# leejaeyong7/nerfacc

Hardware: AMD Instinct MI355X
Metric: rays/sec (fwd+bwd) through 128^3 occ-grid, 1M-ray batch (higher is better)
Workload: dtype f32; 1 GPU; cfg2: 1048576 image rays/GPU, 128^3 shell10 occ grid (G=1), step 2*sqrt(3)/1024, sampling+rendering fwd+bwd; rays_per_gpu=1048576, resolution=128, grid=shell10, samples_after_compaction=32244949, parallelism=ray-sharded x1, field=synthetic analytic field, native callbacks (see bench.py NativeField/TorchField)

## Files before the change

include/nerfacc_hip.h:

```cpp
#ifndef NERFACC_HIP_H
#define NERFACC_HIP_H

#include <stdint.h>

#ifdef __cplusplus
extern "C" {
#endif

#define NFA_OK 0
#define NFA_EINVAL (-1)
#define NFA_EHIP (-2)

#define NFA_MAX_GRID_LEVELS 8

typedef void *nfa_stream_t;

#define NFA_ELEM_F32 0
#define NFA_ELEM_F16 1
#define NFA_ELEM_BF16 2

const char *nfa_last_error(void);
#define NFA_VERSION 403
int nfa_version(void);
int nfa_set_tuning(const char *name, const char *value);
int nfa_device_arch(char *buf, int buflen);


int64_t nfa_cumsum_scratch_bytes(int64_t n);
int nfa_exclusive_cumsum_i64(const int64_t *cnts, int64_t n, int64_t *starts, int64_t *total,
                             void *scratch, nfa_stream_t stream);
int nfa_exclusive_cumsum_pairs_i64(const int64_t *cnts, int64_t n, int64_t *packed_info , int64_t *total,
                                   void *scratch, nfa_stream_t stream);
int nfa_exclusive_cumsum_pairs_stats_i64(const int64_t *cnts, int64_t n, int64_t *packed_info ,
                                         int64_t *total_and_stats , void *scratch, nfa_stream_t stream);

int nfa_pack_info(const int64_t *ray_indices, int64_t n, int64_t n_rays, int64_t *packed_info ,
                  int32_t *flags , void *scratch, nfa_stream_t stream);

int nfa_unpack_rows(const void *packed, const int64_t *packed_info , const uint8_t *mask, int64_t n_rays,
                    int64_t n_per_ray, int64_t n_packed, int64_t row_bytes, const void *pad_host, int32_t pad_bytes,
                    void *padded, nfa_stream_t stream);
int nfa_pack_rows(const void *padded, const int64_t *packed_info , const uint8_t *mask, int64_t n_rays,
                  int64_t n_per_ray, int64_t n_packed, int64_t row_bytes, void *packed, nfa_stream_t stream);
int nfa_mask_row_counts(const uint8_t *mask, int64_t n_rows, int64_t n_cols, int64_t *counts, nfa_stream_t stream);

int nfa_pack_bits(const uint8_t *binaries, int64_t n_cells, uint32_t *bits , nfa_stream_t stream);


int nfa_ray_aabb_intersect(const float *rays_o, const float *rays_d, int64_t n_rays,
                           const float *aabbs, int32_t n_aabbs, float near_plane, float far_plane,
                           float miss_value, float *t_mins, float *t_maxs, uint8_t *hits,
                           nfa_stream_t stream);

#define NFA_MAX_EVENT_LEVELS 8
int nfa_ray_events(const float *rays_o, const float *rays_d, int64_t n_rays, const float *aabbs, int32_t n_aabbs,
                   float *t_sorted, int64_t *t_indices, uint8_t *hits, nfa_stream_t stream);

typedef struct nfa_traverse_args {
    int64_t n_rays;
    const float *rays_o;
    const float *rays_d;
    const uint8_t *rays_mask;
    int32_t n_grids;
    int32_t res[3];
    const uint8_t *binaries;
    const float *aabbs;
    const uint8_t *hits;
    const float *t_sorted;
    const int64_t *t_indices;
    const float *near_planes;
    const float *far_planes;
    float step_size;
    float cone_angle;
    int32_t traverse_steps_limit;
    int32_t mode;
    float *iv_vals; int64_t *iv_ray_indices; uint8_t *iv_is_left; uint8_t *iv_is_right;
    int64_t *iv_starts; int64_t *iv_cnts;
    float *sm_vals; int64_t *sm_ray_indices; uint8_t *sm_is_valid;
    float *sm_t_starts; float *sm_t_ends;
    int64_t *sm_starts; int64_t *sm_cnts;
    float *terminate_planes;
    const int32_t *ray_filter;
    int32_t ray_filter_min;
    const uint64_t *bricks;
    const uint32_t *coarse;
    const int32_t *steps_limit_dev;
    const int64_t *n_listed_dev;
    const int32_t *run_if_nonzero;
} nfa_traverse_args;
int nfa_traverse_grids(const nfa_traverse_args *args, nfa_stream_t stream);

int64_t nfa_bricks_words(int32_t n_grids, const int32_t *res);
int nfa_pack_bricks(const uint8_t *binaries, int32_t n_grids, const int32_t *res, uint64_t *bricks,
                    uint32_t *coarse, nfa_stream_t stream);
int64_t nfa_walk_bits_words(int32_t n_grids, const int32_t *res);
int nfa_pack_walk_bits(const uint8_t *binaries, int32_t n_grids, const int32_t *res, uint32_t *bits, nfa_stream_t stream);
int nfa_traverse_runs(const nfa_traverse_args *args, const uint32_t *bits, int32_t *run_cnts, uint64_t *runs,
                      int32_t max_runs, int32_t *overflow_count, float near_hint, const int32_t *ray_order,
                      int64_t n_order, nfa_stream_t stream);
int nfa_bin_rays(const float *rays_o, const float *rays_d, int64_t n_rays, const float *box, int32_t *order,
                 void *scratch, nfa_stream_t stream);
int nfa_alive_rays(const float *opacity, const int64_t *packed_info , int64_t n_samples, float opacity_max,
                   int64_t n_rays, uint8_t *mask, int32_t *alive, int64_t *count, nfa_stream_t stream);
int nfa_testmode_begin(int64_t *alive_count, int32_t *state, int64_t n_rays, int32_t min_samples, int32_t max_samples,
                       int64_t *sm_cnts, int32_t *run_cnts, int64_t *zero_words, int32_t n_zero, nfa_stream_t stream);
int nfa_testmode_alive(const float *opacity, const int64_t *packed_info, int32_t *state, float opacity_max, int64_t n_rays,
                       uint8_t *mask, int32_t *alive, int64_t *count, int32_t count_samples, nfa_stream_t stream);
int nfa_bin_rays_levels(const float *rays_o, const float *rays_d, int64_t n_rays, const float *aabbs, int32_t n_grids,
                        const int32_t *res, float near_plane, int32_t *order, void *scratch,
                        uint64_t *coherence , nfa_stream_t stream);
int nfa_expand_runs(int64_t n_rays, float step_size, const int32_t *run_cnts, const uint64_t *runs,
                    int32_t max_runs, const int64_t *packed_info , float *t_starts,
                    float *t_ends, float *t_mids, int64_t *ray_indices, int64_t capacity, nfa_stream_t stream);
int nfa_fill_ray_indices(int64_t n_rays, const int64_t *packed_info , int64_t *ray_indices,
                         nfa_stream_t stream);
int nfa_traverse_cone_runs(const nfa_traverse_args *args, int32_t *run_cnts, uint64_t *runs, int32_t max_runs,
                           int32_t *overflow_count, const int32_t *ray_order ,
                           int64_t n_order, nfa_stream_t stream);
int nfa_traverse_cone_walk(const nfa_traverse_args *args, const uint32_t *bits, int32_t *run_cnts, uint64_t *runs,
                           int32_t max_runs, int32_t *overflow_count, uint32_t *arena, int32_t arena_capacity,
                           const int32_t *ray_order, int64_t n_order, nfa_stream_t stream);
int nfa_expand_cone_arena(const uint32_t *arena, int32_t n_entries, float step_size, float cone_angle,
                          const int64_t *packed_info , float *t_starts, float *t_ends, int64_t *ray_indices,
                          nfa_stream_t stream);
int nfa_expand_cone_runs(int64_t n_rays, float step_size, float cone_angle, const int32_t *run_cnts,
                         const uint64_t *runs, int32_t max_runs, const int64_t *packed_info, float *t_starts,
                         float *t_ends, int64_t *ray_indices, nfa_stream_t stream);
int nfa_expand_intervals(int64_t n_rays, float step_size, const int32_t *run_cnts, const uint64_t *runs,
                         int32_t max_runs, const int64_t *iv_packed_info , float *vals,
                         int64_t *ray_indices, uint8_t *is_left, uint8_t *is_right, nfa_stream_t stream);


int nfa_grid_cell_points(const int64_t *indices, const float *jitter , int64_t n, const int32_t *res,
                         const float *aabb , float *x , nfa_stream_t stream);
int nfa_grid_ema_update(float *occs, int64_t cell_base, const int64_t *indices, int64_t n, const float *occ,
                        float ema_decay, float *scratch , nfa_stream_t stream);
int64_t nfa_grid_rebinarize_scratch_bytes(void);
int nfa_grid_rebinarize(const float *occs, int32_t n_grids, const int32_t *res, float occ_thre, uint8_t *binaries,
                        uint32_t *walk_bits, void *scratch, nfa_stream_t stream);


void nfa_seg_plan(int64_t n_elems, int64_t n_rays, int64_t *tile_elems, int64_t *n_tiles);
int64_t nfa_seg_table_rows(int64_t n_tiles);
int nfa_seg_build_tiles(const int64_t *packed_info , int64_t n_rays, int64_t n_elems,
                        int64_t tile_elems, int64_t n_tiles, int64_t *tiles ,
                        int32_t *flags, nfa_stream_t stream);

int nfa_packed_scan(int kind, int reverse, const int64_t *packed_info, const int64_t *tiles, int64_t n_tiles,
                    int64_t n_rays, int64_t n_elems, const float *inputs, float *outputs,
                    nfa_stream_t stream);
int nfa_packed_scan_generic(int kind, int reverse, int normalize, const int64_t *packed_info,
                            int64_t n_rays, int64_t n_elems, const float *inputs, float *outputs,
                            nfa_stream_t stream);
int nfa_packed_prod_backward(int kind, const int64_t *packed_info, const int64_t *tiles, int64_t n_tiles,
                             int64_t n_rays, int64_t n_elems, const float *inputs,
                             const float *outputs, const float *grad_outputs, float *grad_inputs,
                             nfa_stream_t stream);

int nfa_render_from_density_fwd(const float *t_starts, const float *t_ends, const float *sigmas,
                                const float *prefix_trans , const int64_t *packed_info,
                                const int64_t *tiles, int64_t n_tiles, int64_t n_rays, int64_t n_elems,
                                float *weights, float *trans, float *alphas, nfa_stream_t stream);
int nfa_render_from_alpha_fwd(const float *alphas, const float *prefix_trans, const int64_t *packed_info,
                              const int64_t *tiles, int64_t n_tiles, int64_t n_rays, int64_t n_elems,
                              float *weights, float *trans, nfa_stream_t stream);
int nfa_render_from_density_bwd(const float *t_starts, const float *t_ends, const float *trans,
                                const float *alphas, const float *g_weights, const float *g_trans,
                                const float *g_alphas, const int64_t *packed_info, const int64_t *tiles, int64_t n_tiles,
                                int64_t n_rays, int64_t n_elems, float *grad_sigmas, float *grad_x,
                                nfa_stream_t stream);
int nfa_density_cdf_rows_fwd(const float *t_starts, const float *t_ends, const float *sigmas, const int64_t *packed_info,
                             const int64_t *tiles, int64_t n_tiles, int64_t n_rays, int64_t n_elems, int32_t row_len,
                             float *trans, float *alphas, float *cdfs , nfa_stream_t stream);
int nfa_density_cdf_rows_bwd(const float *t_starts, const float *t_ends, const float *trans, const float *alphas,
                             const float *g_cdfs , const int64_t *packed_info, const int64_t *tiles,
                             int64_t n_tiles, int64_t n_rays, int64_t n_elems, int32_t row_len, float *grad_sigmas,
                             nfa_stream_t stream);
int nfa_render_from_alpha_bwd(const float *alphas, const float *trans, const float *g_weights,
                              const float *g_trans, const int64_t *packed_info, const int64_t *tiles, int64_t n_tiles,
                              int64_t n_rays, int64_t n_elems, float *grad_alphas, nfa_stream_t stream);

int nfa_render_visibility(const float *t_starts, const float *t_ends, const float *sigmas_or_alphas,
                          const float *prefix_trans, float early_stop_eps, float alpha_thre,
                          const int64_t *packed_info, const int64_t *tiles, int64_t n_tiles, int64_t n_rays,
                          int64_t n_elems, uint8_t *vis, int64_t *vis_cnts, nfa_stream_t stream);
int nfa_render_visibility_cs(const float *t_starts, float step, const float *sigmas, const float *prefix_trans,
                             float early_stop_eps, float alpha_thre, const int64_t *packed_info, const int64_t *tiles,
// ... 298 lines not shown
```

nerfacc_amd/_backend.py:

```python
from __future__ import annotations

import ctypes as C
import os
import threading
from typing import Optional

import torch

from . import _build

_lock = threading.Lock()
_lib: Optional[C.CDLL] = None

_vp, _i64, _i32, _f32, _u64, _int = C.c_void_p, C.c_int64, C.c_int32, C.c_float, C.c_uint64, C.c_int


class TraverseArgs(C.Structure):
    _fields_ = [
        ("n_rays", _i64), ("rays_o", _vp), ("rays_d", _vp), ("rays_mask", _vp),
        ("n_grids", _i32), ("res", _i32 * 3), ("binaries", _vp), ("aabbs", _vp),
        ("hits", _vp), ("t_sorted", _vp), ("t_indices", _vp),
        ("near_planes", _vp), ("far_planes", _vp),
        ("step_size", _f32), ("cone_angle", _f32), ("traverse_steps_limit", _i32), ("mode", _i32),
        ("iv_vals", _vp), ("iv_ray_indices", _vp), ("iv_is_left", _vp), ("iv_is_right", _vp),
        ("iv_starts", _vp), ("iv_cnts", _vp),
        ("sm_vals", _vp), ("sm_ray_indices", _vp), ("sm_is_valid", _vp),
        ("sm_t_starts", _vp), ("sm_t_ends", _vp), ("sm_starts", _vp), ("sm_cnts", _vp),
        ("terminate_planes", _vp),
        ("ray_filter", _vp), ("ray_filter_min", _i32),
        ("bricks", _vp), ("coarse", _vp),
        ("steps_limit_dev", _vp), ("n_listed_dev", _vp), ("run_if_nonzero", _vp),
    ]


_SIGS = {
    "nfa_exclusive_cumsum_i64": [_vp, _i64, _vp, _vp, _vp, _vp],
    "nfa_exclusive_cumsum_pairs_i64": [_vp, _i64, _vp, _vp, _vp, _vp],
    "nfa_exclusive_cumsum_pairs_stats_i64": [_vp, _i64, _vp, _vp, _vp, _vp],
    "nfa_pack_info": [_vp, _i64, _i64, _vp, _vp, _vp, _vp],
    "nfa_pdf_loss_fwd": [_vp, _vp, _vp, _vp, _i64, _i32, _i32, _f32, _vp, _vp, _vp],
    "nfa_pdf_loss_bwd": [_vp, _vp, _vp, _i64, _i32, _i32, _f32, _vp, _vp, _vp, _vp],
    "nfa_pdf_loss_partials": [_i64, _i32, _i32],
    "nfa_pdf_loss_sum_fwd": [_vp, _vp, _vp, _vp, _i64, _i32, _i32, _f32, _vp, _vp, _vp],
    "nfa_pdf_loss_mean_bwd": [_vp, _vp, _vp, _i64, _i32, _i32, _f32, _vp, _vp, _vp, _vp],
    "nfa_pack_bits": [_vp, _i64, _vp, _vp],
    "nfa_unpack_rows": [_vp, _vp, _vp, _i64, _i64, _i64, _i64, _vp, _i32, _vp, _vp],
    "nfa_pack_rows": [_vp, _vp, _vp, _i64, _i64, _i64, _i64, _vp, _vp],
    "nfa_mask_row_counts": [_vp, _i64, _i64, _vp, _vp],
    "nfa_ray_aabb_intersect": [_vp, _vp, _i64, _vp, _i32, _f32, _f32, _f32, _vp, _vp, _vp, _vp],
    "nfa_ray_events": [_vp, _vp, _i64, _vp, _i32, _vp, _vp, _vp, _vp],
    "nfa_traverse_grids": [C.POINTER(TraverseArgs), _vp],
    "nfa_bricks_words": [_i32, C.POINTER(_i32)],
    "nfa_pack_bricks": [_vp, _i32, C.POINTER(_i32), _vp, _vp, _vp],
    "nfa_walk_bits_words": [_i32, C.POINTER(_i32)],
    "nfa_pack_walk_bits": [_vp, _i32, C.POINTER(_i32), _vp, _vp],
    "nfa_traverse_runs": [C.POINTER(TraverseArgs), _vp, _vp, _vp, _i32, _vp, _f32, _vp, _i64, _vp],
    "nfa_bin_rays": [_vp, _vp, _i64, _vp, _vp, _vp, _vp],
    "nfa_grid_cell_points": [_vp, _vp, _i64, C.POINTER(_i32), _vp, _vp, _vp],
    "nfa_grid_ema_update": [_vp, _i64, _vp, _i64, _vp, _f32, _vp, _vp],
    "nfa_grid_rebinarize_scratch_bytes": [],
    "nfa_grid_rebinarize": [_vp, _i32, C.POINTER(_i32), _f32, _vp, _vp, _vp, _vp],
    "nfa_expand_runs": [_i64, _f32, _vp, _vp, _i32, _vp, _vp, _vp, _vp, _vp, _i64, _vp],
    "nfa_fill_ray_indices": [_i64, _vp, _vp, _vp],
    "nfa_traverse_cone_runs": [C.POINTER(TraverseArgs), _vp, _vp, _i32, _vp, _vp, _i64, _vp],
    "nfa_alive_rays": [_vp, _vp, _i64, _f32, _i64, _vp, _vp, _vp, _vp],
    "nfa_testmode_begin": [_vp, _vp, _i64, _i32, _i32, _vp, _vp, _vp, _i32, _vp],
    "nfa_testmode_alive": [_vp, _vp, _vp, _f32, _i64, _vp, _vp, _vp, _i32, _vp],
    "nfa_traverse_cone_walk": [C.POINTER(TraverseArgs), _vp, _vp, _vp, _i32, _vp, _vp, _i32, _vp, _i64, _vp],
    "nfa_expand_cone_arena": [_vp, _i32, _f32, _f32, _vp, _vp, _vp, _vp, _vp],
    "nfa_bin_rays_levels": [_vp, _vp, _i64, _vp, _i32, C.POINTER(_i32), _f32, _vp, _vp, _vp, _vp],
    "nfa_expand_cone_runs": [_i64, _f32, _f32, _vp, _vp, _i32, _vp, _vp, _vp, _vp, _vp],
    "nfa_expand_intervals": [_i64, _f32, _vp, _vp, _i32, _vp, _vp, _vp, _vp, _vp, _vp],
    "nfa_seg_plan": [_i64, _i64, C.POINTER(_i64), C.POINTER(_i64)],
    "nfa_seg_table_rows": [_i64],
    "nfa_seg_build_tiles": [_vp, _i64, _i64, _i64, _i64, _vp, _vp, _vp],
    "nfa_packed_scan": [_int, _int, _vp, _vp, _i64, _i64, _i64, _vp, _vp, _vp],
    "nfa_packed_scan_generic": [_int, _int, _int, _vp, _i64, _i64, _vp, _vp, _vp],
    "nfa_packed_prod_backward": [_int, _vp, _vp, _i64, _i64, _i64, _vp, _vp, _vp, _vp, _vp],
    "nfa_render_from_density_fwd": [_vp, _vp, _vp, _vp, _vp, _vp, _i64, _i64, _i64, _vp, _vp, _vp, _vp],
    "nfa_render_from_alpha_fwd": [_vp, _vp, _vp, _vp, _i64, _i64, _i64, _vp, _vp, _vp],
    "nfa_render_from_density_bwd": [_vp, _vp, _vp, _vp, _vp, _vp, _vp, _vp, _vp, _i64, _i64, _i64, _vp, _vp, _vp],
    "nfa_density_cdf_rows_fwd": [_vp, _vp, _vp, _vp, _vp, _i64, _i64, _i64, _i32, _vp, _vp, _vp, _vp],
    "nfa_density_cdf_rows_bwd": [_vp, _vp, _vp, _vp, _vp, _vp, _vp, _i64, _i64, _i64, _i32, _vp, _vp],
    "nfa_render_from_alpha_bwd": [_vp, _vp, _vp, _vp, _vp, _vp, _i64, _i64, _i64, _vp, _vp],
    "nfa_render_visibility": [_vp, _vp, _vp, _vp, _f32, _f32, _vp, _vp, _i64, _i64, _i64, _vp, _vp, _vp],
    "nfa_render_visibility_cs": [_vp, _f32, _vp, _vp, _f32, _f32, _vp, _vp, _i64, _i64, _i64, _vp, _vp, _vp],
    "nfa_compact_samples": [_vp, _vp, _vp, _vp, _vp, _i64, _vp, _i64, _i64, _vp, _vp, _vp, _i64, _vp],
    "nfa_accumulate_along_rays": [_vp, _vp, _i32, _vp, _vp, _i64, _i64, _i64, _int, _vp, _vp],
    "nfa_accumulate_along_rays_atomic": [_vp, _vp, _i32, _vp, _i64, _i64, _vp, _vp],
    "nfa_accumulate_along_rays_bwd": [_vp, _vp, _i32, _vp, _vp, _vp, _i64, _i64, _i64, _vp, _vp, _vp],
    "nfa_render_accumulate_fwd": [_vp, _vp, _vp, _vp, _vp, _vp, _i64, _i64, _i64, _vp, _vp, _vp, _vp],
    "nfa_render_accumulate_bwd": [_vp, _vp, _vp, _vp, _vp, _vp, _vp, _vp, _vp, _i64, _i64, _i64, _vp, _vp, _vp],
    "nfa_render_fused_fwd": [_vp, _vp, _vp, _vp, _vp, _vp, _i64, _i64, _i64, _vp, _vp, _vp, _vp, _vp, _vp, _vp],
    "nfa_render_fused_bwd": [_vp] * 13 + [_i64, _i64, _i64, _vp, _vp, _vp],
    "nfa_render_fused_fwd_cs": [_vp, _f32, _vp, _vp, _vp, _vp, _i64, _i64, _i64, _vp, _vp, _vp, _vp, _vp, _vp, _vp],
    "nfa_render_fused_bwd_cs": [_vp, _f32] + [_vp] * 11 + [_i64, _i64, _i64, _vp, _vp, _vp],
    "nfa_render_raw_fwd": [_vp] * 5 + [_i32, _f32, _i32, _vp, _vp, _i64, _i64, _i64] + [_vp] * 9,
    "nfa_render_raw_bwd": [_vp] * 5 + [_i32, _f32, _i32] + [_vp] * 9 + [_i64, _i64, _i64, _vp, _vp, _vp],
    "nfa_render_raw_fwd_t": [_i32] + [_vp] * 5 + [_i32, _f32, _i32, _vp, _vp, _i64, _i64, _i64] + [_vp] * 9,
    "nfa_render_raw_bwd_t": [_i32] + [_vp] * 5 + [_i32, _f32, _i32] + [_vp] * 9 + [_i64, _i64, _i64, _vp, _vp, _vp],
    "nfa_render_sdf_fwd": [_vp] * 6 + [_i32, _vp, _f32, _i32, _vp, _vp, _i64, _i64, _i64] + [_vp] * 7,
    "nfa_render_sdf_bwd": [_vp] * 6 + [_i32, _vp, _f32, _i32] + [_vp] * 9 + [_i64, _i64, _i64] + [_vp] * 5,
    "nfa_render_step_accumulate": [_vp, _vp, _vp, _vp, _vp, _vp, _i64, _i64, _i64, _f32, _vp, _vp, _vp, _vp, _vp],
    "nfa_distortion_fwd": [_vp, _vp, _vp, _vp, _vp, _i64, _i64, _i64, _vp, _vp, _vp, _vp],
    "nfa_distortion_bwd": [_vp] * 8 + [_i64, _i64, _i64, _vp, _vp, _vp, _vp],
    "nfa_importance_sampling": [_vp, _vp, _vp, _i64, _i64, _i64, _int, _u64, _u64, _vp, _vp, _vp],
    "nfa_importance_sampling_t": [_vp, _vp, _vp, _i64, _i64, _i64, _int, _u64, _u64, _vp, _vp, _int, _f32, _f32, _vp, _vp, _vp],
    "nfa_importance_sampling_packed": [_vp, _vp, _vp, _i64, _i64, _vp, _vp, _int, _u64, _u64, _vp, _vp, _vp, _vp, _vp, _vp, _vp],
    "nfa_searchsorted": [_vp, _vp, _vp, _i64, _i64, _i64, _vp, _vp, _i64, _vp, _vp, _vp],
    "nfa_opencv_lens_undistortion": [_vp, _vp, _i64, _i32, _i64, _f32, _i32, _vp, _vp],
    "nfa_opencv_lens_undistortion_fisheye": [_vp, _vp, _i64, _i32, _i64, _f32, _i32, _vp, _vp],
    "nfa_hashgrid_fwd": [_vp, _vp, _i64, _i32, _i32, _i32, _vp, _vp, _vp, _i64, _vp, _vp],
    "nfa_hashgrid_bwd": [_vp, _vp, _vp, _i64, _i32, _i32, _i32, _vp, _vp, _vp, _i64, _vp, _vp, _vp],
    "nfa_sh_fwd": [_vp, _i64, _i32, _vp, _vp],
    "nfa_sh_bwd": [_vp, _vp, _i64, _i32, _vp, _vp],
    "nfa_hashgrid_fwd_t": [_i32, _vp, _vp, _i64, _i32, _i32, _i32, _vp, _vp, _vp, _i64, _vp, _vp],
    "nfa_hashgrid_bwd_t": [_i32, _vp, _vp, _vp, _i64, _i32, _i32, _i32, _vp, _vp, _vp, _i64, _vp, _vp, _vp],
    "nfa_hashgrid_bwd_bwd": [_vp, _vp, _vp, _vp, _i64, _i32, _i32, _i32, _vp, _vp, _vp, _i64, _vp, _vp, _vp, _vp],
    "nfa_hashgrid_bwd_bwd_t": [_i32, _vp, _vp, _vp, _vp, _i64, _i32, _i32, _i32, _vp, _vp, _vp, _i64, _vp, _vp, _vp, _vp],
    "nfa_hashgrid_sorted_scratch_bytes": [_i64, _i32, _i32],
    "nfa_hashgrid_bwd_sorted": [_i32, _vp, _vp, _vp, _i64, _i32, _i32, _i32, _vp, _vp, _vp, _i64, _vp, _vp, _vp, _i64, _vp],
    "nfa_hashgrid_bwd_bwd_sorted": [_i32, _vp, _vp, _vp, _vp, _i64, _i32, _i32, _i32, _vp, _vp, _vp, _i64, _vp, _vp, _vp, _vp, _i64, _vp],
    "nfa_hashgrid_fwd_i": [_i32, _i32, _vp, _vp, _i64, _i32, _i32, _i32, _vp, _vp, _vp, _i64, _vp, _vp],
    "nfa_hashgrid_bwd_i": [_i32, _i32, _vp, _vp, _vp, _i64, _i32, _i32, _i32, _vp, _vp, _vp, _i64, _vp, _vp, _vp],
    "nfa_hashgrid_bwd_bwd_i": [_i32, _i32, _vp, _vp, _vp, _vp, _i64, _i32, _i32, _i32, _vp, _vp, _vp, _i64, _vp, _vp, _vp, _vp],
    "nfa_hashgrid_bwd_sorted_i": [_i32, _i32, _vp, _vp, _vp, _i64, _i32, _i32, _i32, _vp, _vp, _vp, _i64, _vp, _vp, _vp, _i64, _vp],
    "nfa_hashgrid_bwd_bwd_sorted_i": [_i32, _i32, _vp, _vp, _vp, _vp, _i64, _i32, _i32, _i32, _vp, _vp, _vp, _i64, _vp, _vp, _vp, _vp,
                                      _i64, _vp],
    "nfa_hashgrid_fwd_d": [_i32, _i32, _i32, _vp, _vp, _i64, _i32, _i32, _i32, _vp, _vp, _vp, _i64, _vp, _vp],
    "nfa_hashgrid_bwd_d": [_i32, _i32, _i32, _vp, _vp, _vp, _i64, _i32, _i32, _i32, _vp, _vp, _vp, _i64, _vp, _vp, _vp],
    "nfa_hashgrid_bwd_sorted_d": [_i32, _i32, _i32, _vp, _vp, _vp, _i64, _i32, _i32, _i32, _vp, _vp, _vp, _i64, _vp, _vp, _vp, _i64,
                                  _vp],
    "nfa_hashgrid_sorted_scratch_bytes_d": [_i32, _i64, _i32, _i32],
    "nfa_sh_fwd_t": [_i32, _vp, _i64, _i32, _vp, _vp],
    "nfa_sh_bwd_t": [_i32, _vp, _vp, _i64, _i32, _vp, _vp],
    "nfa_planegrid_fwd": [_i32, _i32, _i32, _vp, _vp, _i64, _i32, _i32, C.POINTER(_i32), _vp, _vp],
    "nfa_planegrid_bwd": [_i32, _i32, _i32, _vp, _vp, _vp, _i64, _i32, _i32, C.POINTER(_i32), _vp, _vp, _vp],
    "nfa_planereg_partials": [_i32, _i32, _i32, C.POINTER(_i32)],
    "nfa_planereg_fwd": [_i32, _vp, _i32, _i32, C.POINTER(_i32), _vp, _i64, _vp, _vp],
    "nfa_planereg_bwd": [_i32, _vp, _i32, _i32, C.POINTER(_i32), _vp, _vp, _vp],
    "nfa_vmgrid_fwd": [_i32, _i32, _vp, _vp, _i64, _i32, C.POINTER(_i32), _vp, _vp],
    "nfa_vmgrid_bwd": [_i32, _i32, _vp, _vp, _vp, _i64, _i32, C.POINTER(_i32), _vp, _vp, _vp],
    "nfa_vmgrid_resample": [_vp, C.POINTER(_i32), _vp, C.POINTER(_i32), _i32, _vp],
    "nfa_vmreg_partials": [_i32, C.POINTER(_i32)],
    "nfa_vmreg_fwd": [_vp, _i32, C.POINTER(_i32), _vp, _i64, _vp, _vp, _vp],
    "nfa_vmreg_bwd": [_vp, _i32, C.POINTER(_i32), _vp, _vp, _vp, _vp],
    "nfa_sinenc_fwd": [_i32, _vp, _vp, _vp, _i64, _i32, _i32, _i32, _i32, _vp, _vp],
    "nfa_sinenc_bwd": [_i32, _vp, _vp, _vp, _vp, _i64, _i32, _i32, _i32, _i32, _vp, _vp, _vp],
    "nfa_sinenc_bwd_bwd": [_i32, _vp, _vp, _vp, _vp, _i64, _i32, _i32, _i32, _i32, _vp, _vp, _vp],
    "nfa_sample_positions_fwd": [_vp, _vp, _vp, _vp, _vp, _i64, _i64, _i64, _vp, _vp, _i32, _i32, _vp, _vp, _vp, _vp],
    "nfa_sample_positions_bwd": [_vp] * 9 + [_i64, _i64, _i64, _i64, _vp, _vp, _i32, _i32, _vp, _vp, _vp, _vp, _vp, _vp],
    "nfa_generate_rays_fwd": [_vp, _vp, _i32, _vp, _i64, _i64, _vp, _i64, _vp, _i64, _vp, _i32, _i64, _i32, _i32, _f32, _i32, _f32, _i32,
                              _vp, _vp, _vp],
    "nfa_generate_rays_bwd": [_vp, _vp, _i32, _vp, _vp, _i64, _i64, _vp, _i64, _vp, _i64, _vp, _i32, _i64, _i32, _i32, _f32, _i32, _f32,
                              _i32, _vp, _vp, _vp, _i64, _i32, _vp, _vp, _vp],
    "nfa_generate_rays_chunk": [],
    "nfa_cumsum_scratch_bytes": [_i64],
    "nfa_last_error": [],
    "nfa_version": [],
    "nfa_set_tuning": [C.c_char_p, C.c_char_p],
    "nfa_device_arch": [C.c_char_p, _int],
}
_RESTYPES = {"nfa_grid_rebinarize_scratch_bytes": _i64, "nfa_hashgrid_sorted_scratch_bytes": _i64, "nfa_hashgrid_sorted_scratch_bytes_d": _i64, "nfa_planereg_partials": _i64, "nfa_vmreg_partials": _i64, "nfa_bricks_words": _i64, "nfa_walk_bits_words": _i64, "nfa_pdf_loss_partials": _i64, "nfa_cumsum_scratch_bytes": _i64, "nfa_seg_table_rows": _i64, "nfa_seg_plan": None, "nfa_last_error": C.c_char_p}

EXPORTED_SYMBOLS = tuple(_SIGS)


def library_path() -> str:
    return _build.LIB_PATH


def load() -> C.CDLL:
    global _lib
    if _lib is not None:
        return _lib
    with _lock:
        if _lib is not None:
            return _lib
        path = _build.LIB_PATH
        if _build.is_stale() and _build.hipcc() is not None:
            path = _build.build()
        if not os.path.exists(path):
            raise RuntimeError(
                "nerfacc_amd: libnerfacc_hip.so is missing and hipcc is not available to build it. "
                "There is no CPU fallback for the native ops.")
        lib = C.CDLL(path)
        for name, argtypes in _SIGS.items():
            fn = getattr(lib, name)
            fn.argtypes = argtypes
            fn.restype = _RESTYPES[name] if name in _RESTYPES else _int
        if lib.nfa_version() != ABI_VERSION:
            raise RuntimeError(f"nerfacc_amd: {path} was built from include/nerfacc_hip.h version {lib.nfa_version()}, these "
                               f"bindings are written for {ABI_VERSION}: rebuild the library (nerfacc_amd._build.build(force=True))")
        _lib = lib
    return _lib


ABI_VERSION = 403


ELEM_CODES = {torch.float32: 0, torch.float16: 1, torch.bfloat16: 2}
INTERP_CODES = {"Linear": 0, "Smoothstep": 1}
PLANE_REDUCE_CODES = {"product": 0, "sum": 1}
VM_REDUCE_CODES = {"concat": 0, "sum": 1}


def set_tuning(name: str, value: Optional[str]) -> None:
    call("nfa_set_tuning", name.encode(), None if value is None else str(value).encode())


class NativeError(RuntimeError):
    """Counterpart of the RuntimeError TORCH_CHECK raises in the reference."""


def call(name: str, *args) -> None:
    lib = load()
    rc = getattr(lib, name)(*args)
    if rc != 0:
        msg = lib.nfa_last_error()
        raise NativeError(f"{name}: {msg.decode() if msg else rc}")


def call_group(name: str, fn) -> None:
    fn()


def ptr(t: Optional[torch.Tensor]):
    return None if t is None else t.data_ptr()


_RAW_STREAM = getattr(torch._C, "_cuda_getCurrentRawStream", None)
_CUR_DEVICE = getattr(torch._C, "_cuda_getDevice", None)


def stream() -> int:
    if _RAW_STREAM is not None and _CUR_DEVICE is not None:
        return _RAW_STREAM(_CUR_DEVICE())
    return torch.cuda.current_stream().cuda_stream


def require_device(*tensors: Optional[torch.Tensor]) -> torch.device:
    dev = None
    for t in tensors:
        if t is None:
            continue
        if not t.is_cuda:
            raise NotImplementedError(
                "nerfacc_amd: this op runs only on a ROCm device (the reference has no CPU "
                "implementation of its native ops either); got a tensor on " + str(t.device))
        if dev is None:
            dev = t.device
        elif t.device != dev:
            raise RuntimeError(f"nerfacc_amd: tensors on different devices ({dev} vs {t.device})")
    if dev is None:
        raise RuntimeError("nerfacc_amd: no tensor argument")
    return dev


def seg_plan(n_elems: int, n_rays: int = 0):
    t, n = _i64(0), _i64(0)
    load().nfa_seg_plan(n_elems, n_rays, C.byref(t), C.byref(n))
    return int(t.value), int(n.value)


def cumsum_scratch(n: int, device) -> torch.Tensor:
    nbytes = ((max(n, 1) + 2047) // 2048 + 1) * 8
    return torch.empty(nbytes // 8, dtype=torch.int64, device=device)
```

nerfacc_amd/_segments.py:

```python
from __future__ import annotations

import ctypes
import weakref
from dataclasses import dataclass
from typing import Optional

import torch
from torch import Tensor

from . import _backend as B


@dataclass
class SegInfo:
    packed_info: Tensor
    n_rays: int
    n_elems: int
    tiles: Optional[Tensor]
    contiguous: bool
    sorted_indices: bool = True
    n_tiles: int = 0
    trusted: bool = False


_ATTR = "_nfa_seg"
_ATTR_RI = "_nfa_seg_from_ray_indices"


def _build_tiles(packed_info: Tensor, n_elems: int, trusted: bool) -> SegInfo:
    dev = B.require_device(packed_info)
    n_rays = packed_info.shape[0]
    with torch.cuda.device(dev):
        tile_elems, n_tiles = B.seg_plan(n_elems, n_rays)
        tiles = torch.empty((int(B.load().nfa_seg_table_rows(n_tiles)), 2), dtype=torch.int64, device=dev)
        flag = None if trusted else torch.empty(1, dtype=torch.int32, device=dev)
        B.call("nfa_seg_build_tiles", B.ptr(packed_info), n_rays, n_elems, tile_elems, n_tiles, B.ptr(tiles), B.ptr(flag),
               B.stream())
        ok = True if trusted else (int(flag.item()) == 0)
    return SegInfo(packed_info, n_rays, n_elems, tiles if ok else None, ok, n_tiles=n_tiles, trusted=trusted)


def seginfo_from_packed(packed_info: Tensor, n_elems: int, trusted: bool = False) -> SegInfo:
    assert packed_info.dim() == 2 and packed_info.shape[-1] == 2, "packed_info must be 2-D with shape (B, 2)."
    cached = getattr(packed_info, _ATTR, None)
    if cached is not None and cached[0] == packed_info._version and cached[1] == n_elems:
        return cached[2]
    pi = packed_info
    if pi.dtype != torch.int64 or not pi.is_contiguous():
        pi = pi.to(torch.int64).contiguous()
    info = _build_tiles(pi, n_elems, trusted)
    try:
        setattr(packed_info, _ATTR, (packed_info._version, n_elems, info))
    except Exception:
        pass
    return info


def tag_trusted(packed_info: Tensor, n_elems: int) -> SegInfo:
    return seginfo_from_packed(packed_info, n_elems, trusted=True)


def pack_info_native(ray_indices: Tensor, n_rays: int):
    dev = B.require_device(ray_indices)
    ri = ray_indices if (ray_indices.dtype == torch.int64 and ray_indices.is_contiguous()) else \
        ray_indices.to(torch.int64).contiguous()
    with torch.cuda.device(dev):
        packed = torch.empty((n_rays, 2), dtype=torch.int64, device=dev)
        flag = torch.empty(1, dtype=torch.int32, device=dev)
        scratch = B.cumsum_scratch(n_rays, dev)
        B.call("nfa_pack_info", B.ptr(ri), ri.numel(), n_rays, B.ptr(packed), B.ptr(flag), B.ptr(scratch), B.stream())
    return packed, flag


def seginfo_from_ray_indices(ray_indices: Tensor, n_rays: int) -> SegInfo:
    assert ray_indices.dim() == 1, "ray_indices must be a 1D tensor with shape (n_samples)."
    assert n_rays is not None, "n_rays must be provided"
    cached = getattr(ray_indices, _ATTR_RI, None)
    if cached is not None and cached[0] == ray_indices._version and cached[1] == n_rays:
        return cached[2]
    packed, flag = pack_info_native(ray_indices, n_rays)
    info = _build_tiles(packed, ray_indices.numel(), trusted=True)
    info.sorted_indices = int(flag.item()) == 0
    try:
        setattr(ray_indices, _ATTR_RI, (ray_indices._version, n_rays, info))
    except Exception:
        pass
    return info


def tag_ray_indices(ray_indices: Tensor, n_rays: int, info: SegInfo) -> None:
    setattr(ray_indices, _ATTR_RI, (ray_indices._version, n_rays, info))


def resolve(n_elems: int, packed_info: Optional[Tensor], ray_indices: Optional[Tensor],
            n_rays: Optional[int]) -> Optional[SegInfo]:
    if packed_info is not None:
        return seginfo_from_packed(packed_info, n_elems)
    if ray_indices is not None:
        if n_rays is None:
            n_rays = int(ray_indices.max().item()) + 1 if ray_indices.numel() else 0
        return seginfo_from_ray_indices(ray_indices, n_rays)
    return None


_ATTR_CS = "_nfa_const_step"


def tag_const_step(t_starts: Tensor, t_ends: Tensor, step: float) -> None:
    tag = (t_ends._version, weakref.ref(t_starts), t_starts.data_ptr(), t_starts._version, ctypes.c_float(float(step)).value)
    try:
        setattr(t_ends, _ATTR_CS, tag)
    except Exception:
        pass


def const_step_of(t_starts: Optional[Tensor], t_ends: Optional[Tensor]) -> Optional[float]:
    tag = getattr(t_ends, _ATTR_CS, None) if t_ends is not None else None
    if tag is None or t_starts is None:
        return None
    te_version, ts_ref, ts_ptr, ts_version, step = tag
    if t_ends._version != te_version or ts_ref() is not t_starts:
        return None
    if t_starts.data_ptr() != ts_ptr or t_starts._version != ts_version:
        return None
    for t in (t_starts, t_ends):
        if not (t.is_cuda and t.dtype == torch.float32 and t.dim() == 1 and t.is_contiguous()):
            return None
    if t_starts.shape != t_ends.shape or not (0.0 < step < float("inf")):
        return None
    return step


_UNIFORM: "dict[tuple, SegInfo]" = {}


def uniform_seginfo(n_rows: int, row_len: int, device: torch.device) -> SegInfo:
    key = (int(n_rows), int(row_len), device.type, device.index)
    info = _UNIFORM.get(key)
    if info is None:
        starts = torch.arange(n_rows, dtype=torch.int64, device=device) * row_len
        packed = torch.stack([starts, torch.full_like(starts, row_len)], dim=-1)
        info = _build_tiles(packed, n_rows * row_len, trusted=True)
        setattr(packed, _ATTR, (packed._version, n_rows * row_len, info))
        if len(_UNIFORM) >= 6:
            _UNIFORM.pop(next(iter(_UNIFORM)))
        _UNIFORM[key] = info
    return info


def batched_native(*tensors: Optional[Tensor]) -> Optional[SegInfo]:
    ref = None
    for t in tensors:
        if t is None:
            continue
        if not t.is_cuda or t.dtype != torch.float32 or t.dim() < 1:
            return None
        if ref is None:
            ref = t
        elif t.shape != ref.shape:
            return None
    if ref is None or ref.numel() == 0:
        return None
    return uniform_seginfo(ref.numel() // ref.shape[-1], ref.shape[-1], ref.device)
```

nerfacc_amd/csrc/grid.hip:

```cpp
#include <stdarg.h>

#include "common.hip.h"
#include "march.h"

namespace nfa {

static thread_local char g_err[512] = "";
void set_error(const char *fmt, ...)
{
    va_list ap;
    va_start(ap, fmt);
    vsnprintf(g_err, sizeof(g_err), fmt, ap);
    va_end(ap);
}

struct TuningKnob { char name[32]; char value[64]; };
static TuningKnob g_knobs[8];
static int g_n_knobs = 0;
const char *tuning_env(const char *name)
{
    for (int i = 0; i < g_n_knobs; ++i)
        if (strcmp(g_knobs[i].name, name) == 0) return g_knobs[i].value[0] ? g_knobs[i].value : nullptr;
    return nullptr;
}


__global__ __launch_bounds__(256) void ray_aabb_kernel(const float *__restrict__ rays_o,
                                                       const float *__restrict__ rays_d, int64_t n_rays,
                                                       const float *__restrict__ aabbs, int32_t n_aabbs,
                                                       float near, float far, float miss,
                                                       float *__restrict__ t_mins, float *__restrict__ t_maxs,
                                                       uint8_t *__restrict__ hits)
{
    const int64_t numel = n_rays * n_aabbs;
    for (int64_t tid = (int64_t)blockIdx.x * blockDim.x + threadIdx.x; tid < numel;
         tid += (int64_t)blockDim.x * gridDim.x) {
        const int64_t r = tid / n_aabbs;
        const int32_t g = (int32_t)(tid - r * n_aabbs);
        const float o[3] = {rays_o[3 * r], rays_o[3 * r + 1], rays_o[3 * r + 2]};
        const float inv[3] = {1.0f / rays_d[3 * r], 1.0f / rays_d[3 * r + 1], 1.0f / rays_d[3 * r + 2]};
        float tmin, tmax;
        const bool hit = slab_test(o, inv, aabbs + 6 * g, aabbs + 6 * g + 3, near, far, tmin, tmax);
        t_mins[tid] = hit ? tmin : miss;
        t_maxs[tid] = hit ? tmax : miss;
        hits[tid] = hit ? 1 : 0;
    }
}

template <int G>
__global__ __launch_bounds__(256) void ray_events_kernel(const float *__restrict__ rays_o, const float *__restrict__ rays_d,
                                                         int64_t n_rays, const float *__restrict__ aabbs,
                                                         float *__restrict__ t_sorted, int64_t *__restrict__ t_indices,
                                                         uint8_t *__restrict__ hits)
{
    const float inf = __builtin_inff();
    for (int64_t r = (int64_t)blockIdx.x * blockDim.x + threadIdx.x; r < n_rays; r += (int64_t)blockDim.x * gridDim.x) {
        const float o[3] = {rays_o[3 * r], rays_o[3 * r + 1], rays_o[3 * r + 2]};
        const float inv[3] = {1.0f / rays_d[3 * r], 1.0f / rays_d[3 * r + 1], 1.0f / rays_d[3 * r + 2]};
        float v[2 * G];
        int32_t id[2 * G];
#pragma unroll
        for (int g = 0; g < G; ++g) {
            float tmin, tmax;
            const bool hit = slab_test(o, inv, aabbs + 6 * g, aabbs + 6 * g + 3, -inf, inf, tmin, tmax);
            v[g] = hit ? tmin : inf;
            v[G + g] = hit ? tmax : inf;
            hits[r * G + g] = hit ? 1 : 0;
        }
#pragma unroll
        for (int k = 0; k < 2 * G; ++k) id[k] = k;
#pragma unroll
        for (int i = 1; i < 2 * G; ++i) {
#pragma unroll
            for (int j = i; j > 0; --j) {
                const bool sw = v[j - 1] > v[j];
                const float a = v[j - 1], b = v[j];
                const int32_t ia = id[j - 1], ib = id[j];
                v[j - 1] = sw ? b : a; v[j] = sw ? a : b;
                id[j - 1] = sw ? ib : ia; id[j] = sw ? ia : ib;
            }
        }
#pragma unroll
        for (int k = 0; k < 2 * G; ++k) {
            t_sorted[r * (2 * G) + k] = v[k];
            t_indices[r * (2 * G) + k] = (int64_t)id[k];
        }
    }
}



enum { EMIT_NONE = 0, EMIT_API = 1, EMIT_DIRECT = 2, EMIT_RUNS = 3 };


struct RayState {
    float t_last;
    int32_t continuous;
    int32_t n_intervals;
    int32_t n_samples;
    int32_t brick_id;
    uint32_t brick_lo, brick_hi;
    int32_t n_runs, run_len;
};

struct SpanState {
    float tdist[3], delta[3];
    int32_t step[3], cur[3], overflow[3];
    float this_tmax;
    int32_t level;
    int32_t cells_left;
};

__device__ __forceinline__ int32_t brick_index(const nfa_traverse_args &a, const SpanState &sp)
{
    const int32_t by = (a.res[1] + 3) >> 2, bz = (a.res[2] + 3) >> 2, bx = (a.res[0] + 3) >> 2;
    const int32_t brick_base = sp.level * bx * by * bz;
    return brick_base + (int32_t)mad_u24(mad_u24((uint32_t)sp.cur[0] >> 2, (uint32_t)by, (uint32_t)sp.cur[1] >> 2), (uint32_t)bz, (uint32_t)sp.cur[2] >> 2);
}

__device__ __forceinline__ void span_begin(const nfa_traverse_args &a, const float o[3], const float d[3], const float inv[3],
                                           int32_t level, float this_tmin, float this_tmax, RayState &st, SpanState &sp)
{
    const float eps = 1e-6f;
    if (!st.continuous) st.t_last = fast_forward(st.t_last, this_tmin, a.step_size, a.cone_angle);

    const float *bmin = a.aabbs + 6 * level, *bmax = bmin + 3;
#pragma unroll
    for (int ax = 0; ax < 3; ++ax) {
        const float resf = (float)a.res[ax];
        const float extent = bmax[ax] - bmin[ax];
        const float voxel = extent / resf;
        const float ray_start = o[ax] + d[ax] * (this_tmin + eps);
        const float ray_end = o[ax] + d[ax] * (this_tmax - eps);
        int32_t c = (int32_t)(((ray_start - bmin[ax]) / extent) * resf);
        int32_t f = (int32_t)(((ray_end - bmin[ax]) / extent) * resf);
        c = max(0, min(c, a.res[ax] - 1));
        f = max(0, min(f, a.res[ax] - 1));
        const int32_t start_index = c + (d[ax] > 0.0f ? 1 : 0);
        const float tmax_ax = ((bmin[ax] + (((float)start_index * voxel) - ray_start)) * inv[ax]) + this_tmin;
        const float step_f = (d[ax] == 0.0f) ? 0.0f : (d[ax] > 0.0f ? 1.0f : -1.0f);
        sp.tdist[ax] = (d[ax] == 0.0f) ? this_tmax : tmax_ax;
        sp.step[ax] = (int32_t)step_f;
        const float delta_tmp = voxel * inv[ax] * step_f;
        sp.delta[ax] = (d[ax] == 0.0f) ? this_tmax : delta_tmp;
        sp.cur[ax] = c;
        sp.overflow[ax] = f + sp.step[ax];
    }
    sp.this_tmax = this_tmax;
    sp.level = level;
    sp.cells_left = a.res[0] + a.res[1] + a.res[2] + 3;
    if (a.bricks != nullptr) {
        const int32_t bid = brick_index(a, sp);
        if (bid != st.brick_id) {
            st.brick_id = bid;
            const unsigned long long w = a.bricks[bid];
// ... 187 lines not shown
    {
        tid = ray;
        if (ray_masked(a, ro, tid)) return false;
        if (a.ray_filter != nullptr && a.ray_filter[tid] <= a.ray_filter_min) return false;
        const bool ray_ok = ray_load(a, tid, near_plane, far_plane, o, d);
#pragma unroll
        for (int ax = 0; ax < 3; ++ax) inv[ax] = 1.0f / d[ax];
        st.t_last = near_plane; st.continuous = 0; st.n_samples = 0;
        st.brick_id = -1; st.n_runs = 0; st.run_len = 0;
        ev = ray_ok ? 0 : 2 * a.n_grids;
        return true;
    }
    __device__ __forceinline__ bool next_span()
    {
        int32_t level;
        float this_tmin, this_tmax;
        if (!nfa::next_span<FUSED>(a, tid, o, inv, near_plane, far_plane, ev, level, this_tmin, this_tmax)) return false;
        span_begin(a, o, d, inv, level, this_tmin, this_tmax, st, sp);
        return true;
    }
    __device__ __forceinline__ int cell()
    {
        if (!span_cell<EMIT_RUNS, false, true, true>(a, tid, 0, 0, sp, st, ro)) return RF_WALK;
        return (a.traverse_steps_limit > 0 && st.n_samples >= a.traverse_steps_limit) ? RF_FINISH : RF_SPAN;
    }
    __device__ __forceinline__ void finish() { run_ray_close(a, ro, tid, st.t_last, st.n_samples, st.n_runs); }
};
template <bool FUSED>
__global__ __launch_bounds__(256) void traverse_refill_kernel(const nfa_traverse_args a, const RunOut ro, const int32_t chunk,
                                                              const int32_t min_busy)
{
    SpanState sp;
    BrickWalker<FUSED> w{a, ro, 0, 0, 0.0f, 0.0f, {0.0f, 0.0f, 0.0f}, {0.0f, 0.0f, 0.0f}, {0.0f, 0.0f, 0.0f}, RayState{0.0f, 0, 0, 0, -1, 0u, 0u, 0, 0}, sp};
    refill_schedule(w, ro.order, ro.order ? ro.n_order : a.n_rays, (int64_t)blockIdx.x * (blockDim.x >> 6) + (threadIdx.x >> 6), chunk, min_busy);
}

constexpr int CS_THREADS = 256;
constexpr int CS_ITEMS = 8;
constexpr int CS_BLOCK = CS_THREADS * CS_ITEMS;

__device__ __forceinline__ int64_t block_excl_scan_i64(int64_t v, int64_t &block_total, int64_t *lds )
{
    const int lane = lane_id(), wave = threadIdx.x >> 6;
    const int64_t incl = wave_incl_sum_i64(v);
    if (lane == 63) lds[wave] = incl;
    __syncthreads();
    int64_t wave_off = 0, tot = 0;
#pragma unroll
    for (int w = 0; w < CS_THREADS / 64; ++w) {
        const int64_t x = lds[w];
        if (w < wave) wave_off += x;
        tot += x;
    }
    __syncthreads();
    block_total = tot;
    return wave_off + incl - v;
}

__global__ __launch_bounds__(CS_THREADS) void cumsum_partials_kernel(const int64_t *__restrict__ in, int64_t n,
                                                                      int64_t in_stride, int64_t *__restrict__ partials)
{
    __shared__ int64_t lds[8];
    const int64_t base = (int64_t)blockIdx.x * CS_BLOCK + (int64_t)threadIdx.x * CS_ITEMS;
    int64_t s = 0;
#pragma unroll
    for (int k = 0; k < CS_ITEMS; ++k)
        if (base + k < n) s += in[(base + k) * in_stride];
    int64_t tot;
    block_excl_scan_i64(s, tot, lds);
    if (threadIdx.x == 0) partials[blockIdx.x] = tot;
}

__global__ __launch_bounds__(CS_THREADS) void cumsum_spine_kernel(int64_t *partials, int64_t n_blocks, int64_t *total)
{
    __shared__ int64_t lds[8];
    int64_t carry = 0;
    for (int64_t base = 0; base < n_blocks; base += CS_THREADS) {
        const int64_t i = base + threadIdx.x;
        const int64_t v = i < n_blocks ? partials[i] : 0;
        int64_t tot;
        const int64_t ex = block_excl_scan_i64(v, tot, lds);
        if (i < n_blocks) partials[i] = carry + ex;
        carry += tot;
    }
    if (threadIdx.x == 0 && total) *total = carry;
}

template <bool SPINE>
__global__ __launch_bounds__(CS_THREADS) void cumsum_final_kernel(const int64_t *__restrict__ in, int64_t n,
                                                                   int64_t in_stride,
                                                                   const int64_t *__restrict__ partials,
                                                                   int64_t *__restrict__ out, int pairs,
                                                                   int64_t *__restrict__ total,
                                                                   unsigned long long *__restrict__ stats = nullptr)
{
    __shared__ int64_t lds[8];
    int64_t block_off = 0;
    if (SPINE) {
        int64_t before = 0;
        for (int64_t j = threadIdx.x; j < (int64_t)blockIdx.x; j += CS_THREADS) before += partials[j];
        block_excl_scan_i64(before, block_off, lds);
    } else {
        block_off = partials[blockIdx.x];
    }
    const int64_t base = (int64_t)blockIdx.x * CS_BLOCK + (int64_t)threadIdx.x * CS_ITEMS;
    int64_t v[CS_ITEMS];
    int64_t s = 0;
#pragma unroll
    for (int k = 0; k < CS_ITEMS; ++k) {
        v[k] = (base + k < n) ? in[(base + k) * in_stride] : 0;
        s += v[k];
    }
    int64_t tot;
    int64_t run = block_off + block_excl_scan_i64(s, tot, lds);
    if (SPINE && total && blockIdx.x == gridDim.x - 1 && threadIdx.x == 0) *total = block_off + tot;
    if (SPINE && stats && (blockIdx.x & 7) == 0) {
        int64_t m = 0;
#pragma unroll
        for (int k = 0; k < CS_ITEMS; ++k) m = v[k] > m ? v[k] : m;
        for (int off = 1; off < 8; off <<= 1) { const int64_t u = __shfl_xor(m, off, 64); m = u > m ? u : m; }
        int64_t gm = (lane_id() & 7) == 0 ? m : 0;
        for (int off = 8; off < 64; off <<= 1) gm += __shfl_xor(gm, off, 64);
        if (lane_id() == 0) atomicAdd(&stats[0], (unsigned long long)gm);
        if (threadIdx.x == 0) atomicAdd(&stats[1], (unsigned long long)tot);
    }
#pragma unroll
    for (int k = 0; k < CS_ITEMS; ++k) {
        if (base + k < n) {
            if (pairs) { out[2 * (base + k)] = run; out[2 * (base + k) + 1] = v[k]; }
            else out[base + k] = run;
        }
        run += v[k];
    }
}

static int run_cumsum(const int64_t *in, int64_t n, int64_t in_stride, int64_t *out, int pairs, int64_t *total,
                      void *scratch, hipStream_t s, unsigned long long *stats = nullptr)
{
    const int64_t n_blocks = ceil_div64(n > 0 ? n : 1, CS_BLOCK);
    int64_t *partials = reinterpret_cast<int64_t *>(scratch);
    hipLaunchKernelGGL(cumsum_partials_kernel, dim3((unsigned)n_blocks), dim3(CS_THREADS), 0, s, in, n, in_stride, partials);
    if (n_blocks <= 2048) {
        hipLaunchKernelGGL(cumsum_final_kernel<true>, dim3((unsigned)n_blocks), dim3(CS_THREADS), 0, s, in, n, in_stride, partials,
                           out, pairs, total, stats);
    } else {
        hipLaunchKernelGGL(cumsum_spine_kernel, dim3(1), dim3(CS_THREADS), 0, s, partials, n_blocks, total);
        hipLaunchKernelGGL(cumsum_final_kernel<false>, dim3((unsigned)n_blocks), dim3(CS_THREADS), 0, s, in, n, in_stride, partials,
                           out, pairs, nullptr, nullptr);
    }
    NFA_CHECK_LAUNCH("exclusive_cumsum_i64");
    return NFA_OK;
}

__global__ __launch_bounds__(256) void pack_hist_kernel(const int64_t *__restrict__ ray_indices, int64_t n,
                                                        int64_t n_rays, unsigned long long *__restrict__ packed,
                                                        int32_t *__restrict__ flags)
{
    const int lane = lane_id();
    for (int64_t base = ((int64_t)blockIdx.x * blockDim.x + threadIdx.x) - lane; base < n;
         base += (int64_t)blockDim.x * gridDim.x) {
        const int64_t i = base + lane;
        const bool valid = i < n;
        const int64_t r = valid ? ray_indices[i] : -1;
        int64_t prev = __shfl_up(r, 1, NFA_WAVE);
        if (lane == 0) prev = (i > 0 && valid) ? ray_indices[i - 1] : r;
        const bool in_range = valid && r >= 0 && r < n_rays;
        if (valid && (!in_range || r < prev)) atomicOr(flags, 1);
        const bool head = valid && (lane == 0 || r != prev);
        const unsigned long long heads = __ballot(head);
        const unsigned long long live = __ballot(valid);
        if (head && in_range) {
            const unsigned long long later = (lane == 63) ? 0ull : (heads >> (lane + 1));
            const int next = later ? (lane + 1 + __builtin_ctzll(later)) : (int)__builtin_popcountll(live);
            atomicAdd(&packed[2 * r + 1], (unsigned long long)(next - lane));
        }
    }
}

__global__ void zero_i64_kernel(int64_t *p, int64_t n, int32_t *flags)
{
    for (int64_t i = (int64_t)blockIdx.x * blockDim.x + threadIdx.x; i < n; i += (int64_t)blockDim.x * gridDim.x) p[i] = 0;
    if (flags && blockIdx.x == 0 && threadIdx.x == 0) *flags = 0;
}

__global__ __launch_bounds__(256) void pack_bits_kernel(const uint8_t *__restrict__ b, int64_t n, uint32_t *__restrict__ bits)
{
    const int lane = lane_id();
    for (int64_t base = ((int64_t)blockIdx.x * blockDim.x + threadIdx.x) - lane; base < n;
         base += (int64_t)blockDim.x * gridDim.x) {
        const int64_t i = base + lane;
        const unsigned long long m = __ballot(i < n && b[i] != 0);
        if (lane == 0) bits[base >> 5] = (uint32_t)m;
        if (lane == 32 && base + 32 < n) bits[(base >> 5) + 1] = (uint32_t)(m >> 32);
    }
}

}

using namespace nfa;

extern "C" {

const char *nfa_last_error(void) { return g_err; }
int nfa_version(void) { return NFA_VERSION; }
int nfa_set_tuning(const char *name, const char *value)
{
    NFA_REQUIRE(name && strlen(name) > 0 && strlen(name) < sizeof(g_knobs[0].name), "set_tuning: bad name");
    NFA_REQUIRE(!value || strlen(value) < sizeof(g_knobs[0].value), "set_tuning: value too long");
    int i = 0;
    while (i < g_n_knobs && strcmp(g_knobs[i].name, name) != 0) ++i;
    if (i == g_n_knobs) {
        NFA_REQUIRE(g_n_knobs < (int)(sizeof(g_knobs) / sizeof(g_knobs[0])), "set_tuning: too many knobs");
        strcpy(g_knobs[g_n_knobs++].name, name);
    }
    strcpy(g_knobs[i].value, value ? value : "");
    return NFA_OK;
}

int nfa_device_arch(char *buf, int buflen)
{
    int dev = 0;
    hipDeviceProp_t prop;
    if (hipGetDevice(&dev) != hipSuccess || hipGetDeviceProperties(&prop, dev) != hipSuccess) {
        set_error("no HIP device");
        return NFA_EHIP;
    }
    snprintf(buf, buflen, "%s", prop.gcnArchName);
    return NFA_OK;
}

int64_t nfa_cumsum_scratch_bytes(int64_t n) { return (ceil_div64(n > 0 ? n : 1, CS_BLOCK) + 1) * 8; }

int nfa_exclusive_cumsum_i64(const int64_t *cnts, int64_t n, int64_t *starts, int64_t *total, void *scratch,
                             nfa_stream_t stream)
{
    NFA_REQUIRE(n >= 0 && scratch && (n == 0 || (cnts && starts)), "exclusive_cumsum_i64: bad arguments");
    return run_cumsum(cnts, n, 1, starts, 0, total, scratch, as_stream(stream));
}

int nfa_exclusive_cumsum_pairs_i64(const int64_t *cnts, int64_t n, int64_t *packed_info, int64_t *total, void *scratch,
                                   nfa_stream_t stream)
{
    NFA_REQUIRE(n >= 0 && scratch && (n == 0 || (cnts && packed_info)), "exclusive_cumsum_pairs_i64: bad arguments");
    return run_cumsum(cnts, n, 1, packed_info, 1, total, scratch, as_stream(stream));
}

int nfa_exclusive_cumsum_pairs_stats_i64(const int64_t *cnts, int64_t n, int64_t *packed_info, int64_t *total_and_stats,
                                         void *scratch, nfa_stream_t stream)
{
    NFA_REQUIRE(n >= 0 && scratch && total_and_stats && (n == 0 || (cnts && packed_info)),
                "exclusive_cumsum_pairs_stats_i64: bad arguments");
    return run_cumsum(cnts, n, 1, packed_info, 1, total_and_stats, scratch, as_stream(stream),
                      reinterpret_cast<unsigned long long *>(total_and_stats + 1));
}

int nfa_pack_info(const int64_t *ray_indices, int64_t n, int64_t n_rays, int64_t *packed_info, int32_t *flags,
                  void *scratch, nfa_stream_t stream)
{
    NFA_REQUIRE(n >= 0 && n_rays >= 0 && flags && scratch, "pack_info: bad arguments");
    NFA_REQUIRE(n_rays == 0 || packed_info, "pack_info: packed_info is null");
    NFA_REQUIRE(n == 0 || ray_indices, "pack_info: ray_indices is null");
    hipStream_t s = as_stream(stream);
    hipLaunchKernelGGL(zero_i64_kernel, dim3(grid_1d(2 * n_rays + 1, 256)), dim3(256), 0, s, packed_info, 2 * n_rays, flags);
    if (n > 0 && n_rays > 0)
        hipLaunchKernelGGL(pack_hist_kernel, dim3(grid_1d(n, 256)), dim3(256), 0, s, ray_indices, n, n_rays,
                           reinterpret_cast<unsigned long long *>(packed_info), flags);
    NFA_CHECK_LAUNCH("pack_info");
    if (n_rays == 0) return NFA_OK;
    return run_cumsum(packed_info + 1, n_rays, 2, packed_info, 1, nullptr, scratch, s);
}

int nfa_pack_bits(const uint8_t *binaries, int64_t n_cells, uint32_t *bits, nfa_stream_t stream)
{
    NFA_REQUIRE(n_cells >= 0 && (n_cells == 0 || (binaries && bits)), "pack_bits: bad arguments");
    if (n_cells == 0) return NFA_OK;
    hipLaunchKernelGGL(pack_bits_kernel, dim3(grid_1d(n_cells, 256)), dim3(256), 0, as_stream(stream), binaries, n_cells, bits);
    NFA_CHECK_LAUNCH("pack_bits");
    return NFA_OK;
}

int nfa_ray_aabb_intersect(const float *rays_o, const float *rays_d, int64_t n_rays, const float *aabbs,
                           int32_t n_aabbs, float near_plane, float far_plane, float miss_value, float *t_mins,
                           float *t_maxs, uint8_t *hits, nfa_stream_t stream)
{
    NFA_REQUIRE(n_rays >= 0 && n_aabbs >= 0, "ray_aabb_intersect: negative size");
    if (n_rays * (int64_t)n_aabbs == 0) return NFA_OK;
    NFA_REQUIRE(rays_o && rays_d && aabbs && t_mins && t_maxs && hits, "ray_aabb_intersect: null pointer");
    hipLaunchKernelGGL(ray_aabb_kernel, dim3(grid_1d(n_rays * n_aabbs, 256)), dim3(256), 0, as_stream(stream), rays_o,
                       rays_d, n_rays, aabbs, n_aabbs, near_plane, far_plane, miss_value, t_mins, t_maxs, hits);
    NFA_CHECK_LAUNCH("ray_aabb_intersect");
    return NFA_OK;
}

int nfa_ray_events(const float *rays_o, const float *rays_d, int64_t n_rays, const float *aabbs, int32_t n_aabbs,
                   float *t_sorted, int64_t *t_indices, uint8_t *hits, nfa_stream_t stream)
{
    NFA_REQUIRE(n_rays >= 0 && n_aabbs >= 1 && n_aabbs <= NFA_MAX_EVENT_LEVELS, "ray_events: 1..NFA_MAX_EVENT_LEVELS boxes");
    if (n_rays == 0) return NFA_OK;
    NFA_REQUIRE(rays_o && rays_d && aabbs && t_sorted && t_indices && hits, "ray_events: null pointer");
    const dim3 grid(grid_1d(n_rays, 256)), block(256);
    hipStream_t s = as_stream(stream);
    static constexpr decltype(&ray_events_kernel<1>) kernels[NFA_MAX_EVENT_LEVELS] = {
        ray_events_kernel<1>, ray_events_kernel<2>, ray_events_kernel<3>, ray_events_kernel<4>,
        ray_events_kernel<5>, ray_events_kernel<6>, ray_events_kernel<7>, ray_events_kernel<8>};
    hipLaunchKernelGGL(kernels[n_aabbs - 1], grid, block, 0, s, rays_o, rays_d, n_rays, aabbs, t_sorted, t_indices, hits);
    NFA_CHECK_LAUNCH("ray_events");
    return NFA_OK;
}

int nfa_traverse_grids(const nfa_traverse_args *pa, nfa_stream_t stream)
{
    NFA_REQUIRE(pa != nullptr, "traverse_grids: null args");
    const nfa_traverse_args &a = *pa;
    NFA_REQUIRE(a.n_rays >= 0 && a.n_rays < (int64_t)1 << 31, "traverse_grids: n_rays out of range");
    if (a.n_rays == 0) return NFA_OK;
    NFA_REQUIRE(a.mode >= 0 && a.mode <= 2, "traverse_grids: mode must be 0, 1 or 2");
    NFA_REQUIRE(a.rays_o && a.rays_d && a.binaries && a.aabbs && a.near_planes && a.far_planes,
                "traverse_grids: null input pointer");
    NFA_REQUIRE(a.n_grids >= 1 && a.res[0] > 0 && a.res[1] > 0 && a.res[2] > 0, "traverse_grids: bad grid shape");
    NFA_REQUIRE((int64_t)a.res[0] * a.res[1] * a.res[2] < (int64_t)1 << 31, "traverse_grids: grid level too large");
    const bool fused = !a.t_sorted && !a.t_indices && !a.hits;
    NFA_REQUIRE(fused || (a.t_sorted && a.t_indices && a.hits),
                "traverse_grids: t_sorted, t_indices and hits must be given together");
    NFA_REQUIRE(!fused || a.n_grids == 1, "traverse_grids: in-kernel intersection supports one grid; pass t_sorted/t_indices/hits");
    NFA_REQUIRE(a.mode != 2 || a.traverse_steps_limit > 0,
                "traverse_steps_limit must be > 0 when over_allocate is true");
    const bool has_iv = a.iv_cnts != nullptr, has_sm = a.sm_cnts != nullptr;
    NFA_REQUIRE(has_iv || has_sm, "traverse_grids: nothing to compute");
    const bool direct = a.sm_t_starts != nullptr;
    hipStream_t s = as_stream(stream);
    if (a.mode == 0) {
        if (has_iv && has_sm) launch_traverse<EMIT_NONE, true, true>(a, fused, s);
        else if (has_sm) launch_traverse<EMIT_NONE, false, true>(a, fused, s);
        else launch_traverse<EMIT_NONE, true, false>(a, fused, s);
    } else {
        NFA_REQUIRE(!has_iv || (a.iv_vals && a.iv_ray_indices && a.iv_is_left && a.iv_is_right && a.iv_starts),
                    "traverse_grids: interval outputs missing");
        NFA_REQUIRE(!has_sm || a.sm_starts, "traverse_grids: sample starts missing");
        if (direct) {
            NFA_REQUIRE(!has_iv && has_sm && a.sm_t_ends,
                        "traverse_grids: direct emission needs sm_t_starts, sm_t_ends and no intervals");
            launch_traverse<EMIT_DIRECT, false, true>(a, fused, s);
        } else {
            NFA_REQUIRE(!has_sm || (a.sm_vals && a.sm_ray_indices && a.sm_is_valid), "traverse_grids: sample outputs missing");
            if (has_iv && has_sm) launch_traverse<EMIT_API, true, true>(a, fused, s);
            else if (has_sm) launch_traverse<EMIT_API, false, true>(a, fused, s);
            else launch_traverse<EMIT_API, true, false>(a, fused, s);
        }
    }
    NFA_CHECK_LAUNCH("traverse_grids");
    return NFA_OK;
}

int nfa_traverse_cone_runs(const nfa_traverse_args *pa, int32_t *run_cnts, uint64_t *runs, int32_t max_runs,
                           int32_t *overflow_count, const int32_t *ray_order, int64_t n_order, nfa_stream_t stream)
{
    NFA_REQUIRE(pa != nullptr, "traverse_cone_runs: null args");
    const nfa_traverse_args &a = *pa;
    NFA_REQUIRE(a.n_rays >= 0 && a.n_rays < (int64_t)1 << 31, "traverse_cone_runs: n_rays out of range");
    NFA_REQUIRE(overflow_count, "traverse_cone_runs: overflow_count is null");
    hipStream_t s = as_stream(stream);
    if (hipMemsetAsync(overflow_count, 0, sizeof(int32_t), s) != hipSuccess) { set_error("traverse_cone_runs: memset failed"); return NFA_EHIP; }
    if (a.n_rays == 0) return NFA_OK;
    NFA_REQUIRE(a.step_size > 0.0f && a.cone_angle > 0.0f, "traverse_cone_runs: needs step_size > 0 and cone_angle > 0");
    NFA_REQUIRE(a.mode == 0 || a.mode == 2, "traverse_cone_runs: mode must be 0 (all rays) or 2 (rays_mask + traverse_steps_limit)");
    NFA_REQUIRE(a.mode != 2 || a.traverse_steps_limit > 0, "traverse_steps_limit must be > 0 when over_allocate is true");
    NFA_REQUIRE(a.rays_o && a.rays_d && a.binaries && a.aabbs && a.near_planes && a.far_planes && a.sm_cnts && !a.iv_cnts &&
                    run_cnts && runs, "traverse_cone_runs: null pointer (or interval outputs requested)");
    NFA_REQUIRE(max_runs >= 1 && max_runs <= 32, "traverse_cone_runs: max_runs must be in [1, 32]");
    NFA_REQUIRE(a.n_grids >= 1 && a.res[0] > 0 && a.res[1] > 0 && a.res[2] > 0, "traverse_cone_runs: bad grid shape");
    NFA_REQUIRE((int64_t)a.res[0] * a.res[1] * a.res[2] < (int64_t)1 << 31, "traverse_cone_runs: grid level too large");
    const bool fused = !a.t_sorted && !a.t_indices && !a.hits;
    NFA_REQUIRE(fused || (a.t_sorted && a.t_indices && a.hits), "traverse_cone_runs: t_sorted, t_indices and hits must be given together");
    NFA_REQUIRE(!fused || a.n_grids == 1, "traverse_cone_runs: in-kernel intersection supports one grid");
    RunOut ro;
    ro.run_cnts = run_cnts;
    ro.runs = reinterpret_cast<unsigned long long *>(runs);
    ro.max_runs = max_runs;
    ro.overflow = overflow_count;
    ro.order = ray_order;
    ro.n_order = ray_order ? n_order : a.n_rays;
    NFA_REQUIRE(!ray_order || (n_order >= 0 && n_order <= a.n_rays), "traverse_cone_runs: n_order out of range");
    if (ray_order && n_order == 0) return NFA_OK;
    const RefillPlan plan = refill_plan(ro.n_order, a.traverse_steps_limit);
    if (plan.refill) {
        const unsigned grid = (unsigned)ceil_div64(ceil_div64(ro.n_order, plan.chunk), 4);
        if (fused) hipLaunchKernelGGL((traverse_refill_kernel<true>), dim3(grid), dim3(256), 0, s, a, ro, (int32_t)plan.chunk, plan.min_busy);
        else       hipLaunchKernelGGL((traverse_refill_kernel<false>), dim3(grid), dim3(256), 0, s, a, ro, (int32_t)plan.chunk, plan.min_busy);
    } else {
        launch_traverse<EMIT_RUNS, false, true>(a, fused, s, ro);
    }
    NFA_CHECK_LAUNCH("traverse_cone_runs");
    return NFA_OK;
}

}
```

nerfacc_amd/csrc/segscan.hip:

```cpp
#include <stdlib.h>

#include "common.hip.h"
#include "samples.h"

namespace nfa {

constexpr int SE = 4;
constexpr int SQ = SE / 4;
constexpr int SEG_CHUNK = 64 * SE;
#ifndef NFA_SEG_TILE_ROWS
#define NFA_SEG_TILE_ROWS 256
#endif
constexpr int64_t SEG_TILE_ROWS = NFA_SEG_TILE_ROWS;
#ifndef NFA_VIS_EXP_FREE
#define NFA_VIS_EXP_FREE 1
#endif
#ifndef NFA_SEG_WAVES_PER_BLOCK
#define NFA_SEG_WAVES_PER_BLOCK 4
#endif
constexpr int SEG_WAVES_PER_BLOCK = NFA_SEG_WAVES_PER_BLOCK;

__global__ __launch_bounds__(256) void seg_build_tiles_kernel(const int64_t *__restrict__ packed_info, int64_t n_rays,
                                                              int64_t n_elems, int64_t tile_elems, int64_t n_tiles,
                                                              longlong2 *__restrict__ tiles, int32_t *__restrict__ flags)
{
    for (int64_t r = (int64_t)blockIdx.x * blockDim.x + threadIdx.x; r <= n_rays;
         r += (int64_t)blockDim.x * gridDim.x) {
        int64_t b_lo, b_hi, e_first;
        bool bad = false;
        if (r < n_rays) {
            const int64_t s = packed_info[2 * r], n = packed_info[2 * r + 1];
            int64_t s_prev = -1;
            if (r > 0) {
                const int64_t ps = packed_info[2 * r - 2], pn = packed_info[2 * r - 1];
                s_prev = ps;
                bad |= (ps + pn != s);
            }
            bad |= (n < 0) || (s < 0) || (s + n > n_elems);
            if (bad) { if (flags) atomicOr(flags, 1); continue; }
            b_lo = (s_prev < 0) ? 0 : s_prev / tile_elems + (r - 1) / SEG_TILE_ROWS + 1;
            b_hi = s / tile_elems + r / SEG_TILE_ROWS;
            e_first = s;
        } else {
            const int64_t s_prev = n_rays > 0 ? packed_info[2 * n_rays - 2] : -1;
            const int64_t n_prev = n_rays > 0 ? packed_info[2 * n_rays - 1] : 0;
            b_lo = (s_prev < 0) ? 0 : s_prev / tile_elems + (n_rays - 1) / SEG_TILE_ROWS + 1;
            b_hi = n_tiles;
            e_first = (s_prev < 0) ? 0 : s_prev + n_prev;
            if (s_prev > n_elems) { if (flags) atomicOr(flags, 1); continue; }
        }
        for (int64_t b = b_lo; b <= b_hi && b <= n_tiles; ++b) tiles[b] = make_longlong2(r, e_first);
    }
}

__host__ __device__ inline int64_t seg_table_rows(int64_t n_tiles) { return n_tiles + 1; }

struct F4 { float v[SE]; };

struct Pos {
    int64_t c;
    int32_t off;
    int32_t safe;
    bool valid[SE];
    bool any, all;
    int32_t d_lo, d_hi;
    bool qany[SQ], qall[SQ];
    __device__ __forceinline__ int64_t p0() const { return c + off; }
};

template <bool VEC>
__device__ __forceinline__ void ld4(const float *__restrict__ p, const Pos &q, F4 &out)
{
    const float *b = p + q.c;
    if (VEC) {
#pragma unroll
        for (int h = 0; h < SQ; ++h) {
            const nfa_v4f v = *reinterpret_cast<const nfa_v4f *>(b + (q.qany[h] ? q.off + 4 * h : q.safe));
            out.v[4 * h] = v.x; out.v[4 * h + 1] = v.y; out.v[4 * h + 2] = v.z; out.v[4 * h + 3] = v.w;
        }
    } else {
#pragma unroll
        for (int j = 0; j < SE; ++j) out.v[j] = b[q.valid[j] ? q.off + j : q.safe];
    }
}
__device__ __forceinline__ float sel(const F4 &r, int j, const bool valid[SE], float fill) { return valid[j] ? r.v[j] : fill; }

#define NFA_ELEMENTWISE_PATH() asm volatile("; element-wise path" ::: "memory")
template <bool VEC>
__device__ __forceinline__ void store4(float *__restrict__ p, const Pos &q, const float v[SE])
{
    float *b = p + q.c;
#pragma unroll
    for (int h = 0; h < SQ; ++h) {
        if (VEC && q.qall[h]) {
            store_f4(b + q.off + 4 * h, v[4 * h], v[4 * h + 1], v[4 * h + 2], v[4 * h + 3]);
        } else {
            NFA_ELEMENTWISE_PATH();
#pragma unroll
            for (int j = 4 * h; j < 4 * h + 4; ++j)
                if (q.valid[j]) b[q.off + j] = v[j];
        }
    }
}

struct StepHeads {
    int32_t lh[SE];
    uint32_t acc;
    bool open_prefix;
    bool carry_on_lane_end;
    int32_t carry_lane;
    int32_t ph;
    int32_t rid[SE], prev_rid[SE];
    bool is_head[SE];
};

template <int S>
__device__ __forceinline__ void heads_step(int32_t &ah, uint32_t &acc)
{
    const int32_t uh = dpp_step<S>(-1, ah);
    if (ah < 0) { acc |= 1u << S; ah = uh; }
}

template <int DIR>
__device__ __forceinline__ void resolve_heads(const int32_t hj[SE], const bool valid[SE], int32_t carry_rid, StepHeads &hd)
{
#pragma unroll
    for (int k = 0; k < SE; ++k) {
        const int j = DIR > 0 ? k : SE - 1 - k;
        const int32_t h = valid[j] ? hj[j] : -1;
        hd.is_head[k] = h >= 0;
        hd.lh[k] = (k == 0 || h >= 0) ? h : hd.lh[k - 1 < 0 ? 0 : k - 1];
    }
    int32_t ah = hd.lh[SE - 1];
    uint32_t acc = 0;
    heads_step<0>(ah, acc); heads_step<1>(ah, acc); heads_step<2>(ah, acc);
    heads_step<3>(ah, acc); heads_step<4>(ah, acc); heads_step<5>(ah, acc);
    const int lane = lane_id(), r = lane & 15;
    const uint32_t has_src = (r >= 1 ? 1u : 0u) | (r >= 2 ? 2u : 0u) | (r >= 4 ? 4u : 0u) | (r >= 8 ? 8u : 0u) |
                             ((lane & 16) ? 16u : 0u) | (lane >= 32 ? 32u : 0u);
    hd.acc = acc & has_src;
    int32_t ph = dpp_prev_lane(-1, ah);
    hd.open_prefix = ph < 0;
    if (ph < 0) ph = carry_rid;
    hd.ph = ph;
    int32_t pr = ph;
#pragma unroll
    for (int k = 0; k < SE; ++k) {
        hd.prev_rid[k] = pr;
        hd.rid[k] = hd.lh[k] >= 0 ? hd.lh[k] : ph;
        pr = hd.rid[k];
    }
}

template <int S, int N, class FI, class FC>
__device__ __forceinline__ void values_step(const StepHeads &hd, float av[N], FI identity, FC comb)
{
    const bool take = (hd.acc >> S) & 1u;
#pragma unroll
    for (int ch = 0; ch < N; ++ch) {
        const float uv = dpp_step<S>(identity(ch), av[ch]);
        if (take) av[ch] = comb(ch, uv, av[ch]);
    }
}

template <int N, class FI, class FC>
__device__ __forceinline__ void scan_values(const StepHeads &hd, const float x[SE][N], float carry[N], float incl[SE][N],
                                            float prev[SE][N], FI identity, FC comb)
{
    float li[SE][N];
#pragma unroll
    for (int k = 0; k < SE; ++k)
#pragma unroll
        for (int ch = 0; ch < N; ++ch)
            li[k][ch] = (k == 0 || hd.is_head[k]) ? x[k][ch] : comb(ch, li[k - 1 < 0 ? 0 : k - 1][ch], x[k][ch]);
    float av[N];
#pragma unroll
    for (int ch = 0; ch < N; ++ch) av[ch] = li[SE - 1][ch];
    values_step<0, N>(hd, av, identity, comb); values_step<1, N>(hd, av, identity, comb);
    values_step<2, N>(hd, av, identity, comb); values_step<3, N>(hd, av, identity, comb);
    values_step<4, N>(hd, av, identity, comb); values_step<5, N>(hd, av, identity, comb);
    float pv[N];
#pragma unroll
    for (int ch = 0; ch < N; ++ch) {
        pv[ch] = dpp_prev_lane(identity(ch), av[ch]);
        if (hd.open_prefix) pv[ch] = comb(ch, carry[ch], pv[ch]);
    }
#pragma unroll
    for (int k = 0; k < SE; ++k)
#pragma unroll
        for (int ch = 0; ch < N; ++ch) {
            prev[k][ch] = (k == 0) ? pv[ch] : incl[k - 1 < 0 ? 0 : k - 1][ch];
            incl[k][ch] = hd.lh[k] >= 0 ? li[k][ch] : comb(ch, pv[ch], li[k][ch]);
        }
    const bool open_next = hd.open_prefix && hd.lh[SE - 1] < 0;
#pragma unroll
    for (int ch = 0; ch < N; ++ch) {
        const float nxt = open_next ? comb(ch, carry[ch], av[ch]) : av[ch];
        carry[ch] = lane_value(hd.carry_on_lane_end ? nxt : incl[SE - 1][ch], hd.carry_lane);
    }
}

template <int N, class F>
__device__ __forceinline__ void flush_totals(const StepHeads &hd, const float prev[SE][N], F &&done)
{
    bool f[SE];
    int nf = 0;
#pragma unroll
    for (int k = 0; k < SE; ++k) { f[k] = hd.is_head[k] && hd.prev_rid[k] >= 0; nf += f[k] ? 1 : 0; }
// ... 1809 lines not shown
        if (MODE != SP_NONE) {
            float lo[3], ext[3];
            box_resolve(box, lo, ext);
            if (MODE == SP_SPHERE || MODE == SP_CUBE) sample_point(ro, rd, tsv[j], tev[j], p);
            sample_grad_point<MODE>(p, lo, ext, g);
        }
        const float m = (tsv[j] + tev[j]) / 2.0f;
#pragma unroll
        for (int k = 0; k < 3; ++k) {
            xv[j][k] = g[k];
            xv[j][3 + k] = m * g[k] + dscale * gdv[3 * j + k];
        }
        rt[j] = 0.5f * (rd[0] * g[0] + rd[1] * g[1] + rd[2] * g[2]);
    }
    __device__ __forceinline__ void store_pre(const Pos &) const {}
    __device__ __forceinline__ float x(int j, int ch) const { return xv[j][ch]; }
    __device__ __forceinline__ void emit(int, int64_t, bool, bool, int, int, const float *, const float *) const {}
    __device__ __forceinline__ void store(const Pos &q)
    {
        if (gts) store4<VEC>(gts, q, rt);
        if (gte) store4<VEC>(gte, q, rt);
    }
    __device__ __forceinline__ void put(int rid, const float *t) const
    {
        if (go) { go[3 * (int64_t)rid] = t[0]; go[3 * (int64_t)rid + 1] = t[1]; go[3 * (int64_t)rid + 2] = t[2]; }
        if (gd) { gd[3 * (int64_t)rid] = t[3]; gd[3 * (int64_t)rid + 1] = t[4]; gd[3 * (int64_t)rid + 2] = t[5]; }
    }
    __device__ __forceinline__ void ray_done(int rid, const float t[6]) const { put(rid, t); }
    __device__ __forceinline__ void empty_ray(int rid) const
    {
        const float z[6] = {0, 0, 0, 0, 0, 0};
        put(rid, z);
    }
};

template <bool EXCL, bool PROD>
__global__ __launch_bounds__(256) void generic_scan_kernel(const int64_t *__restrict__ packed_info, int64_t n_rays,
                                                           const float *__restrict__ in, float *__restrict__ out,
                                                           int reverse, int normalize)
{
    const int lane = lane_id();
    const float init = PROD ? 1.0f : 0.0f;
    for (int64_t r = ((int64_t)blockIdx.x * blockDim.x + threadIdx.x) >> 6; r < n_rays;
         r += ((int64_t)blockDim.x * gridDim.x) >> 6) {
        const int64_t s = packed_info[2 * r], n = packed_info[2 * r + 1];
        if (n <= 0) continue;
        float den = 1.0f;
        if (normalize) {
            float tot = init;
            for (int64_t k = lane; k < n; k += 64) tot = PROD ? tot * in[s + k] : tot + in[s + k];
#pragma unroll
            for (int off = 32; off >= 1; off >>= 1) {
                const float u = __shfl_xor(tot, off, 64);
                tot = PROD ? tot * u : tot + u;
            }
            den = fmaxf(tot, 1e-10f);
        }
        float carry = init;
        for (int64_t c = 0; c < n; c += 64) {
            const int64_t k = c + lane;
            const int64_t pos = reverse ? s + n - 1 - k : s + k;
            float v = k < n ? in[pos] : init;
#pragma unroll
            for (int off = 1; off < 64; off <<= 1) {
                const float u = __shfl_up(v, off, 64);
                if (lane >= off) v = PROD ? u * v : u + v;
            }
            v = PROD ? carry * v : carry + v;
            float prevv = __shfl_up(v, 1, 64);
            if (lane == 0) prevv = carry;
            if (k < n) {
                float o = EXCL ? prevv : v;
                if (normalize && !(EXCL && k == 0)) o /= den;
                out[pos] = o;
            }
            carry = __shfl(v, 63, 64);
        }
    }
}

__global__ __launch_bounds__(256) void accumulate_atomic_kernel(const float *__restrict__ w, const float *__restrict__ vals,
                                                                int32_t D, const int64_t *__restrict__ ri, int64_t n_rays,
                                                                int64_t n, float *__restrict__ out)
{
    for (int64_t i = (int64_t)blockIdx.x * blockDim.x + threadIdx.x; i < n * D; i += (int64_t)blockDim.x * gridDim.x) {
        const int64_t e = i / D;
        const int32_t ch = (int32_t)(i - e * D);
        const int64_t r = ri[e];
        if (r < 0 || r >= n_rays) continue;
        const float v = vals ? w[e] * vals[i] : w[e];
        atomicAdd(out + r * D + ch, v);
    }
}

}

using namespace nfa;

#define SEG_COMMON_CHECKS(name)                                                                         \
    NFA_REQUIRE(n_rays >= 0 && n_elems >= 0, name ": negative size");                                   \
    NFA_REQUIRE(n_rays < ((int64_t)1 << 31) - 64, name ": too many rays");                              \
    if (n_elems == 0 && n_rays == 0) return NFA_OK;                                                      \
    NFA_REQUIRE(packed_info && tiles && n_tiles >= 1, name ": packed_info/tiles is null")

static inline bool aligned_quads(const float *p) { return aligned16(p); }
static inline bool aligned_quads(const void *p) { return (reinterpret_cast<uintptr_t>(p) & 7) == 0; }

template <class E, class Make>
static int launch_render_fwd(const char *name, Make &&make, bool own_aligned, const float *t_starts, const float *t_ends, const E *sigmas,
                             const E *rgbs, float *weights, float *trans, float *alphas, float *colors, float *opacities,
                             float *depths, const int64_t *packed_info, const int64_t *tiles, int64_t n_tiles, int64_t n_rays,
                             nfa_stream_t stream)
{
    const bool vec = own_aligned && all_aligned16(t_starts, t_ends, weights, trans, alphas) && aligned_quads(sigmas) && aligned_quads(rgbs);
    dispatch_bool(vec, [&](auto V) {
        auto op = make(V);
        op.ts = t_starts; op.te = t_ends; op.sig = sigmas; op.rgb = rgbs; op.w = weights; op.tr = trans; op.al = alphas;
        op.colors = colors; op.opac = opacities; op.depth = depths;
        launch_seg<1>(op, packed_info, tiles, n_rays, n_tiles, as_stream(stream));
    });
    NFA_CHECK_LAUNCH(name);
    return NFA_OK;
}

template <class E, class Make>
static int launch_render_bwd(const char *name, Make &&make, bool own_aligned, const float *t_starts, const float *t_ends, const E *rgbs,
                             const float *trans, const float *g_colors, const float *g_opacities, const float *g_depths,
                             const float *g_weights, const float *g_trans, const float *g_alphas, E *grad_sigmas, E *grad_rgbs,
                             const int64_t *packed_info, const int64_t *tiles, int64_t n_tiles, int64_t n_rays, nfa_stream_t stream)
{
    const bool vec = own_aligned && all_aligned16(t_starts, t_ends, trans, g_weights, g_trans, g_alphas) && aligned_quads(rgbs) &&
                     aligned_quads(grad_sigmas) && aligned_quads(grad_rgbs);
    const bool extra = g_weights || g_trans || g_alphas;
    dispatch_bool(vec, [&](auto V) {
        dispatch_bool(extra, [&](auto X) {
            auto op = make(V, X);
            op.ts = t_starts; op.te = t_ends; op.rgb = rgbs; op.tr = trans;
            op.gc = g_colors; op.go = g_opacities; op.gd = g_depths; op.gw = g_weights; op.gt = g_trans; op.ga = g_alphas;
            op.gsig = grad_sigmas; op.grgb = grad_rgbs;
            launch_seg<-1>(op, packed_info, tiles, n_rays, n_tiles, as_stream(stream));
        });
    });
    NFA_CHECK_LAUNCH(name);
    return NFA_OK;
}

extern "C" {

void nfa_seg_plan(int64_t n_elems, int64_t n_rays, int64_t *tile_elems, int64_t *n_tiles)
{
    const int64_t t_env = tuning_env("NFA_SEG_TILE") ? atoll(tuning_env("NFA_SEG_TILE")) : 0;
    const int64_t t = t_env > 0 ? t_env : 1024;
    *tile_elems = t;
    *n_tiles = n_elems / t + (n_rays > 0 ? n_rays : 0) / SEG_TILE_ROWS + 1;
}

int64_t nfa_seg_table_rows(int64_t n_tiles) { return seg_table_rows(n_tiles); }

int nfa_seg_build_tiles(const int64_t *packed_info, int64_t n_rays, int64_t n_elems, int64_t tile_elems, int64_t n_tiles,
                        int64_t *tiles, int32_t *flags, nfa_stream_t stream)
{
    NFA_REQUIRE(n_rays >= 0 && n_elems >= 0 && tiles, "seg_build_tiles: bad arguments");
    NFA_REQUIRE(n_rays == 0 || packed_info, "seg_build_tiles: packed_info is null");
    NFA_REQUIRE(n_rays < ((int64_t)1 << 31) - 64, "seg_build_tiles: too many rays");
    NFA_REQUIRE(tile_elems >= 64 && tile_elems % 4 == 0 && n_tiles == n_elems / tile_elems + n_rays / SEG_TILE_ROWS + 1,
                "seg_build_tiles: tile_elems must be a multiple of 4 (>= 64) and n_tiles what nfa_seg_plan returns for (n_elems, n_rays)");
    hipStream_t s = as_stream(stream);
    if (flags && hipMemsetAsync(flags, 0, sizeof(int32_t), s) != hipSuccess) { set_error("seg_build_tiles: memset failed"); return NFA_EHIP; }
    hipLaunchKernelGGL(seg_build_tiles_kernel, dim3(grid_1d(n_rays + 1, 256)), dim3(256), 0, s, packed_info, n_rays,
                       n_elems, tile_elems, n_tiles, reinterpret_cast<longlong2 *>(tiles), flags);
    NFA_CHECK_LAUNCH("seg_build_tiles");
    return NFA_OK;
}

int nfa_packed_scan(int kind, int reverse, const int64_t *packed_info, const int64_t *tiles, int64_t n_tiles, int64_t n_rays,
                    int64_t n_elems, const float *inputs, float *outputs, nfa_stream_t stream)
{
    SEG_COMMON_CHECKS("packed_scan");
    NFA_REQUIRE(kind >= 0 && kind <= 3, "packed_scan: kind must be 0..3");
    if (n_elems == 0) return NFA_OK;
    NFA_REQUIRE(inputs && outputs, "packed_scan: null data pointer");
    hipStream_t s = as_stream(stream);
    const bool vec = all_aligned16(inputs, outputs);
    dispatch_bool(kind & 1, [&](auto EX) {
        dispatch_bool(kind >= 2, [&](auto PR) {
            dispatch_bool(vec, [&](auto V) {
                ScanOp<EX, PR, V> op;
                op.in = inputs; op.out = outputs;
                dispatch_bool(reverse != 0, [&](auto REV) { launch_seg<REV ? -1 : 1>(op, packed_info, tiles, n_rays, n_tiles, s); });
            });
        });
    });
    NFA_CHECK_LAUNCH("packed_scan");
    return NFA_OK;
}

int nfa_packed_scan_generic(int kind, int reverse, int normalize, const int64_t *packed_info, int64_t n_rays,
                            int64_t n_elems, const float *inputs, float *outputs, nfa_stream_t stream)
{
    NFA_REQUIRE(kind >= 0 && kind <= 3 && n_rays >= 0 && n_elems >= 0, "packed_scan_generic: bad arguments");
    if (n_elems == 0 || n_rays == 0) return NFA_OK;
    NFA_REQUIRE(packed_info && inputs && outputs, "packed_scan_generic: null pointer");
    hipStream_t s = as_stream(stream);
    const unsigned grid = grid_1d(n_rays * 64, 256, 1 << 16);
    dispatch_bool(kind & 1, [&](auto EX) {
        dispatch_bool(kind >= 2, [&](auto PR) {
            hipLaunchKernelGGL((generic_scan_kernel<EX, PR>), dim3(grid), dim3(256), 0, s, packed_info, n_rays, inputs, outputs, reverse, normalize);
        });
    });
    NFA_CHECK_LAUNCH("packed_scan_generic");
    return NFA_OK;
}

int nfa_packed_prod_backward(int kind, const int64_t *packed_info, const int64_t *tiles, int64_t n_tiles, int64_t n_rays,
                             int64_t n_elems, const float *inputs, const float *outputs, const float *grad_outputs,
                             float *grad_inputs, nfa_stream_t stream)
{
    SEG_COMMON_CHECKS("packed_prod_backward");
    NFA_REQUIRE(kind == 2 || kind == 3, "packed_prod_backward: kind must be 2 or 3");
    if (n_elems == 0) return NFA_OK;
    NFA_REQUIRE(inputs && outputs && grad_outputs && grad_inputs, "packed_prod_backward: null data pointer");
    hipStream_t s = as_stream(stream);
    const bool vec = all_aligned16(inputs, outputs, grad_outputs, grad_inputs);
    dispatch_bool(kind == 3, [&](auto EX) {
        dispatch_bool(vec, [&](auto V) {
            ProdBwdOp<EX, V> op;
            op.in = inputs; op.outv = outputs; op.g = grad_outputs; op.gin = grad_inputs;
            launch_seg<-1>(op, packed_info, tiles, n_rays, n_tiles, s);
        });
    });
    NFA_CHECK_LAUNCH("packed_prod_backward");
    return NFA_OK;
}

int nfa_render_from_density_fwd(const float *t_starts, const float *t_ends, const float *sigmas,
                                const float *prefix_trans, const int64_t *packed_info, const int64_t *tiles, int64_t n_tiles,
                                int64_t n_rays, int64_t n_elems, float *weights, float *trans, float *alphas,
                                nfa_stream_t stream)
{
    SEG_COMMON_CHECKS("render_from_density_fwd");
    if (n_elems == 0) return NFA_OK;
    NFA_REQUIRE(t_starts && t_ends && sigmas, "render_from_density_fwd: null input");
    hipStream_t s = as_stream(stream);
    const bool vec = all_aligned16(t_starts, t_ends, sigmas, prefix_trans, weights, trans, alphas);
    dispatch_bool(vec, [&](auto V) {
        DensityFwdOp<V> op;
        op.ts = t_starts; op.te = t_ends; op.sig = sigmas; op.prefix = prefix_trans;
        op.w = weights; op.tr = trans; op.al = alphas;
        launch_seg<1>(op, packed_info, tiles, n_rays, n_tiles, s);
    });
    NFA_CHECK_LAUNCH("render_from_density_fwd");
    return NFA_OK;
}

int nfa_render_from_alpha_fwd(const float *alphas, const float *prefix_trans, const int64_t *packed_info,
                              const int64_t *tiles, int64_t n_tiles, int64_t n_rays, int64_t n_elems, float *weights, float *trans,
                              nfa_stream_t stream)
{
    SEG_COMMON_CHECKS("render_from_alpha_fwd");
    if (n_elems == 0) return NFA_OK;
    NFA_REQUIRE(alphas, "render_from_alpha_fwd: null input");
    hipStream_t s = as_stream(stream);
    const bool vec = all_aligned16(alphas, prefix_trans, weights, trans);
    dispatch_bool(vec, [&](auto V) {
        AlphaFwdOp<V> op;
        op.al = alphas; op.prefix = prefix_trans; op.w = weights; op.tr = trans;
        launch_seg<1>(op, packed_info, tiles, n_rays, n_tiles, s);
    });
    NFA_CHECK_LAUNCH("render_from_alpha_fwd");
    return NFA_OK;
}

int nfa_render_from_density_bwd(const float *t_starts, const float *t_ends, const float *trans, const float *alphas,
                                const float *g_weights, const float *g_trans, const float *g_alphas,
                                const int64_t *packed_info, const int64_t *tiles, int64_t n_tiles, int64_t n_rays, int64_t n_elems,
                                float *grad_sigmas, float *grad_x, nfa_stream_t stream)
{
    SEG_COMMON_CHECKS("render_from_density_bwd");
    if (n_elems == 0) return NFA_OK;
    NFA_REQUIRE(t_starts && t_ends && trans && alphas && (grad_sigmas || grad_x), "render_from_density_bwd: null pointer");
    hipStream_t s = as_stream(stream);
    const bool vec = all_aligned16(t_starts, t_ends, trans, alphas, g_weights, g_trans, g_alphas, grad_sigmas, grad_x);
    dispatch_bool(vec, [&](auto V) {
        DensityBwdOp<V> op;
        op.ts = t_starts; op.te = t_ends; op.tr = trans; op.al = alphas;
        op.gw = g_weights; op.gt = g_trans; op.ga = g_alphas; op.gsig = grad_sigmas; op.gx = grad_x;
        launch_seg<-1>(op, packed_info, tiles, n_rays, n_tiles, s);
    });
    NFA_CHECK_LAUNCH("render_from_density_bwd");
    return NFA_OK;
}

int nfa_density_cdf_rows_fwd(const float *t_starts, const float *t_ends, const float *sigmas, const int64_t *packed_info,
                             const int64_t *tiles, int64_t n_tiles, int64_t n_rays, int64_t n_elems, int32_t row_len,
                             float *trans, float *alphas, float *cdfs, nfa_stream_t stream)
{
    SEG_COMMON_CHECKS("density_cdf_rows_fwd");
    if (n_elems == 0) return NFA_OK;
    NFA_REQUIRE(t_starts && t_ends && sigmas && cdfs, "density_cdf_rows_fwd: null pointer");
    NFA_REQUIRE(row_len >= 1 && n_rays * (int64_t)row_len == n_elems, "density_cdf_rows_fwd: n_elems must be n_rays * row_len");
    hipStream_t s = as_stream(stream);
    const bool vec = all_aligned16(t_starts, t_ends, sigmas, trans, alphas);
    dispatch_bool(vec, [&](auto V) {
        DensityFwdOp<V> op;
        op.ts = t_starts; op.te = t_ends; op.sig = sigmas; op.prefix = nullptr;
        op.w = nullptr; op.tr = trans; op.al = alphas; op.cdf = cdfs; op.row_len = row_len;
        launch_seg<1>(op, packed_info, tiles, n_rays, n_tiles, s);
    });
    NFA_CHECK_LAUNCH("density_cdf_rows_fwd");
    return NFA_OK;
}

int nfa_density_cdf_rows_bwd(const float *t_starts, const float *t_ends, const float *trans, const float *alphas,
                             const float *g_cdfs, const int64_t *packed_info, const int64_t *tiles, int64_t n_tiles,
                             int64_t n_rays, int64_t n_elems, int32_t row_len, float *grad_sigmas, nfa_stream_t stream)
{
    SEG_COMMON_CHECKS("density_cdf_rows_bwd");
    if (n_elems == 0) return NFA_OK;
    NFA_REQUIRE(t_starts && t_ends && trans && g_cdfs && grad_sigmas, "density_cdf_rows_bwd: null pointer");
    (void)alphas;
    NFA_REQUIRE(row_len >= 1 && n_rays * (int64_t)row_len == n_elems, "density_cdf_rows_bwd: n_elems must be n_rays * row_len");
    hipStream_t s = as_stream(stream);
    const bool vec = all_aligned16(t_starts, t_ends, trans, alphas, grad_sigmas);
// ... 569 lines not shown
```

nerfacc_amd/estimators/occ_grid.py:

```python
from __future__ import annotations

import ctypes as C
from typing import Callable, List, Optional, Tuple, Union

import torch
from torch import Tensor

from .. import _backend as B
from .._segments import SegInfo, const_step_of, tag_const_step, tag_ray_indices, tag_trusted
from ..grid import _enlarge_aabb, _exclusive_cumsum, _traverse_samples
from .. import volrend as _volrend
from ..volrend import _visibility_native
from .base import AbstractEstimator


class TraversalHandle:

    def __init__(self, tensors, event, key):
        self._tensors, self._event, self.key = tensors, event, key

    def consume(self, stream):
        assert self._tensors is not None, "a TraversalHandle can be consumed once"
        stream.wait_event(self._event)
        tensors, self._tensors = self._tensors, None
        for t in tensors:
            t.record_stream(stream)
        seg = getattr(tensors[3], "_nfa_seg", None)
        if seg is not None and seg[2].tiles is not None:
            seg[2].tiles.record_stream(stream)
        return tensors


class OccGridEstimator(AbstractEstimator):

    DIM: int = 3

    def __init__(self, roi_aabb: Union[List[int], Tensor], resolution: Union[int, List[int], Tensor] = 128,
                 levels: int = 1, **kwargs) -> None:
        super().__init__()
        if "contraction_type" in kwargs:
            raise ValueError("`contraction_type` is not supported anymore for nerfacc >= 0.4.0.")
        if isinstance(resolution, int):
            resolution = [resolution] * self.DIM
        if isinstance(resolution, (list, tuple)):
            resolution = torch.tensor(resolution, dtype=torch.int32)
        assert isinstance(resolution, Tensor), f"Invalid type: {resolution}!"
        assert resolution.shape[0] == self.DIM, f"Invalid shape: {resolution}!"
        if isinstance(roi_aabb, (list, tuple)):
            roi_aabb = torch.tensor(roi_aabb, dtype=torch.float32)
        assert isinstance(roi_aabb, Tensor), f"Invalid type: {roi_aabb}!"
        assert roi_aabb.shape[0] == self.DIM * 2, f"Invalid shape: {roi_aabb}!"

        self.levels = levels
        self.cells_per_lvl = int(resolution.prod().item())
        aabbs = torch.stack([_enlarge_aabb(roi_aabb, 2 ** i) for i in range(levels)], dim=0)
        self.register_buffer("resolution", resolution)
        self.register_buffer("aabbs", aabbs)
        self.register_buffer("occs", torch.zeros(levels * self.cells_per_lvl))
        self.register_buffer("binaries", torch.zeros([levels] + resolution.tolist(), dtype=torch.bool))
        self.register_buffer("grid_coords", _meshgrid3d(resolution).reshape(self.cells_per_lvl, self.DIM),
                             persistent=False)
        self.register_buffer("grid_indices", torch.arange(self.cells_per_lvl), persistent=False)
        self._occs_mean_cache = None
        self._prefetch_stream = None
        self._walk_stats = {}

    def _planes(self, rays_o: Tensor, near_plane: float, far_plane: float):
        key = (rays_o.shape[0], float(near_plane), float(far_plane), rays_o.device, rays_o.dtype)
        cached = getattr(self, "_planes_cache", None)
        if cached is None or cached[0] != key:
            cached = (key, torch.full_like(rays_o[..., 0], fill_value=near_plane),
                      torch.full_like(rays_o[..., 0], fill_value=far_plane))
            self._planes_cache = cached
        return cached[1], cached[2]

    bin_rays: Optional[bool] = None

    def _occs_mean(self) -> float:
        key = (id(self.occs), self.occs.data_ptr(), self.occs._version)
        if self._occs_mean_cache is None or self._occs_mean_cache[0] != key:
            self._occs_mean_cache = (key, float(self.occs.mean().item()))
        return self._occs_mean_cache[1]

    def _traverse(self, rays_o, rays_d, near_plane, far_plane, t_min, t_max, render_step_size, stratified, cone_angle,
                  speculate=True):
        near_planes, far_planes = self._planes(rays_o, near_plane, far_plane)
        if t_min is not None:
            near_planes = torch.clamp(near_planes, min=t_min)
        if t_max is not None:
            far_planes = torch.clamp(far_planes, max=t_max)
        if stratified:
            near_planes = near_planes + torch.rand_like(near_planes) * render_step_size
        use_bins = self.bin_rays
        if use_bins is None and not cone_angle > 0.0:
            use_bins = self._walk_stats.get("max_over_mean", 1.0) > 5.0 and rays_o.shape[0] >= 65536
        return _traverse_samples(rays_o, rays_d, self.binaries, self.aabbs, near_planes, far_planes, render_step_size,
                                 cone_angle, near_hint=near_plane, bin_rays=None if use_bins is None else bool(use_bins),
                                 stats_sink=self._walk_stats, speculate=speculate)

    def _traversal_key(self, rays_o, rays_d, near_plane, far_plane, t_min, t_max, render_step_size, stratified, cone_angle):
        def tid(t):
            return None if t is None else (t.data_ptr(), tuple(t.shape), t._version)
        return (tid(rays_o), tid(rays_d), tid(t_min), tid(t_max), float(near_plane), float(far_plane),
                float(render_step_size), bool(stratified), float(cone_angle), tid(self.binaries), id(self.binaries))

    @torch.no_grad()
    def prefetch_traversal(
        self,
        rays_o: Tensor,
        rays_d: Tensor,
        near_plane: float = 0.0,
        far_plane: float = 1e10,
        t_min: Optional[Tensor] = None,
        t_max: Optional[Tensor] = None,
        render_step_size: float = 1e-3,
        stratified: bool = False,
        cone_angle: float = 0.0,
        wait_for_inputs: bool = True,
    ) -> "TraversalHandle":
        if self._prefetch_stream is None:
            try:
                self._prefetch_stream = torch.cuda.Stream(device=rays_o.device, priority=-1)
            except Exception:
                self._prefetch_stream = torch.cuda.Stream(device=rays_o.device)
        side = self._prefetch_stream
        if wait_for_inputs:
            side.wait_stream(torch.cuda.current_stream(rays_o.device))
        with torch.cuda.stream(side):
            out = self._traverse(rays_o, rays_d, near_plane, far_plane, t_min, t_max, render_step_size, stratified,
                                 cone_angle, speculate=False)
            event = torch.cuda.Event()
            event.record(side)
        key = self._traversal_key(rays_o, rays_d, near_plane, far_plane, t_min, t_max, render_step_size, stratified, cone_angle)
        return TraversalHandle(out, event, key)

    @torch.no_grad()
    def sampling(
        self,
        rays_o: Tensor,
        rays_d: Tensor,
        sigma_fn: Optional[Callable] = None,
        alpha_fn: Optional[Callable] = None,
        near_plane: float = 0.0,
        far_plane: float = 1e10,
        t_min: Optional[Tensor] = None,
        t_max: Optional[Tensor] = None,
        render_step_size: float = 1e-3,
        early_stop_eps: float = 1e-4,
        alpha_thre: float = 0.0,
        stratified: bool = False,
        cone_angle: float = 0.0,
        traversal: Optional["TraversalHandle"] = None,
    ) -> Tuple[Tensor, Tensor, Tensor]:
        if traversal is not None:
            key = self._traversal_key(rays_o, rays_d, near_plane, far_plane, t_min, t_max, render_step_size, stratified, cone_angle)
            if traversal.key != key:
                raise ValueError("nerfacc_amd: the prefetched traversal was made for other rays / planes / step / grid "
                                 "(or the ray / plane tensors were modified in place since)")
            ray_indices, t_starts, t_ends, packed_info = traversal.consume(torch.cuda.current_stream(rays_o.device))
        else:
            ray_indices, t_starts, t_ends, packed_info = self._traverse(
                rays_o, rays_d, near_plane, far_plane, t_min, t_max, render_step_size, stratified, cone_angle)

        if (alpha_thre > 0.0 or early_stop_eps > 0.0) and (sigma_fn is not None or alpha_fn is not None):
            alpha_thre = min(alpha_thre, self._occs_mean())
            seg: SegInfo = tag_trusted(packed_info, t_starts.numel())
            if sigma_fn is not None:
                if t_starts.shape[0] != 0:
                    sigmas = sigma_fn(t_starts, t_ends, ray_indices)
                else:
                    sigmas = torch.empty((0,), device=t_starts.device)
                assert sigmas.shape == t_starts.shape, "sigmas must have shape of (N,)! Got {}".format(sigmas.shape)
                step = const_step_of(t_starts, t_ends) if _volrend.DERIVE_T_ENDS else None
                vis, cnts = _visibility_native(seg, t_starts, t_ends, sigmas, None, early_stop_eps, alpha_thre, True, step=step)
            else:
                if t_starts.shape[0] != 0:
                    alphas = alpha_fn(t_starts, t_ends, ray_indices)
                else:
                    alphas = torch.empty((0,), device=t_starts.device)
                assert alphas.shape == t_starts.shape, "alphas must have shape of (N,)! Got {}".format(alphas.shape)
                vis, cnts = _visibility_native(seg, None, None, alphas, None, early_stop_eps, alpha_thre, True)
            compacted = _compact(seg, vis, cnts, t_starts, t_ends)
            if compacted is not None:
                ray_indices, t_starts, t_ends = compacted
        return ray_indices, t_starts, t_ends

    @torch.no_grad()
    def update_every_n_steps(self, step: int, occ_eval_fn: Callable, occ_thre: float = 1e-2,
                             ema_decay: float = 0.95, warmup_steps: int = 256, n: int = 16) -> None:
        if not self.training:
            raise RuntimeError(
                "You should only call this function only during training. "
                "Please call _update() directly if you want to update the field during inference.")
        if step % n == 0:
            self._update(step=step, occ_eval_fn=occ_eval_fn, occ_thre=occ_thre, ema_decay=ema_decay,
                         warmup_steps=warmup_steps)

    @torch.no_grad()
    def mark_invisible_cells(self, K: Tensor, c2w: Tensor, width: int, height: int, near_plane: float = 0.0,
                             chunk: int = 32 ** 3) -> None:
        assert K.dim() == 3 and K.shape[1:] == (3, 3)
        assert c2w.dim() == 3 and (c2w.shape[1:] == (3, 4) or c2w.shape[1:] == (4, 4))
        assert K.shape[0] == c2w.shape[0] or K.shape[0] == 1
        n_cams = c2w.shape[0]
        rot = c2w[:, :3, :3].transpose(2, 1)
        trans = -rot @ c2w[:, :3, 3:]
        for lvl, indices in enumerate(self._get_all_cells()):
            coords = self.grid_coords[indices]
            lo, hi = self.aabbs[lvl, :3], self.aabbs[lvl, 3:]
            for i in range(0, len(indices), chunk):
                ids = indices[i:i + chunk]
                world = (lo + coords[i:i + chunk] / (self.resolution - 1) * (hi - lo)).T
                uvd = K @ (rot @ world + trans)
                depth = uvd[:, 2]
                uv = uvd[:, :2] / uvd[:, 2:]
                in_image = (depth >= 0) & (uv[:, 0] >= 0) & (uv[:, 0] < width) & (uv[:, 1] >= 0) & (uv[:, 1] < height)
                seen = ((depth >= near_plane) & in_image).sum(0) / n_cams > 0
                too_near = ((depth < near_plane) & in_image).any(0)
                self.occs[lvl * self.cells_per_lvl + ids] = torch.where(seen & ~too_near, 0.0, -1.0)

    @torch.no_grad()
    def _get_all_cells(self) -> List[Tensor]:
        out = []
        for lvl in range(self.levels):
            keep = self.occs[lvl * self.cells_per_lvl + self.grid_indices] >= 0.0
            out.append(self.grid_indices[keep])
        return out

    @torch.no_grad()
    def _sample_uniform_and_occupied_cells(self, n: int) -> List[Tensor]:
        if self.occs.is_cuda and self.levels * self.cells_per_lvl <= self.ONE_READ_MAX_CELLS:
            return self._sample_cells_one_read(n)
        dev, L, cells = self.occs.device, self.levels, self.cells_per_lvl
        out = []
        for lvl in range(L):
            uni = torch.randint(cells, (n,), device=dev)
            uni = uni[self.occs[lvl * cells + uni] >= 0.0]
            occ = torch.nonzero(self.binaries[lvl].flatten())[:, 0]
            if n < len(occ):
                occ = occ[torch.randint(len(occ), (n,), device=dev)]
            out.append(torch.cat([uni, occ], dim=0))
        return out

    ONE_READ_MAX_CELLS = 1 << 27

    @torch.no_grad()
    def _sample_cells_one_read(self, n: int) -> List[Tensor]:
        dev, L, cells = self.occs.device, self.levels, self.cells_per_lvl
        uni = torch.randint(cells, (L, n), device=dev)
        uni_ok = self.occs.view(L, cells).gather(1, uni) >= 0.0
        uni_pos = torch.cumsum(uni_ok, dim=1, dtype=torch.int32)
        occ_flag = self.binaries.view(L, cells)
        occ_pos = torch.cumsum(occ_flag, dim=1, dtype=torch.int32)
        sizes = torch.stack([uni_pos[:, -1], occ_pos[:, -1]], dim=1).tolist()
        out = []
        cell_ids = torch.arange(cells, device=dev)
        for lvl, (n_uni, n_occ) in enumerate(sizes):
            n_uni, n_occ = int(n_uni), int(n_occ)
            if n < n_occ:
                k = torch.randint(n_occ, (n,), device=dev)
                occ = torch.searchsorted(occ_pos[lvl], (k + 1).to(torch.int32))
                n_take = n
            else:
                occ, n_take = None, n_occ
            res = torch.empty(n_uni + n_take + 1, dtype=torch.int64, device=dev)
            dump = n_uni + n_take
            res.scatter_(0, torch.where(uni_ok[lvl], uni_pos[lvl] - 1, dump).long(), uni[lvl])
            if occ is None:
                res.scatter_(0, torch.where(occ_flag[lvl], n_uni + occ_pos[lvl] - 1, dump).long(), cell_ids)
            else:
                res[n_uni:dump] = occ
            out.append(res[:dump])
        return out

    sync_group = None

    @torch.no_grad()
    def _update(self, step: int, occ_eval_fn: Callable, occ_thre: float = 0.01, ema_decay: float = 0.95,
                warmup_steps: int = 256) -> None:
        if step < warmup_steps:
            lvl_indices = self._get_all_cells()
        else:
            lvl_indices = self._sample_uniform_and_occupied_cells(self.cells_per_lvl // 4)
        group = self.sync_group
        if group is not None and torch.distributed.get_world_size(group) > 1:
            cand = torch.full_like(self.occs, float("-inf"))
            for lvl, indices in enumerate(lvl_indices):
                jitter = torch.rand((indices.shape[0], self.DIM), dtype=torch.float32, device=indices.device)
                occ = occ_eval_fn(self._cell_points(lvl, indices, jitter)).squeeze(-1).to(torch.float32)
                cand.scatter_reduce_(0, lvl * self.cells_per_lvl + indices, occ, reduce="amax", include_self=True)
            torch.distributed.all_reduce(cand, op=torch.distributed.ReduceOp.MAX, group=group)
            sampled = cand > float("-inf")
            self.occs = torch.where(sampled, torch.maximum(self.occs * ema_decay, cand), self.occs)
            self._occs_mean_cache = None
        else:
            for lvl, indices in enumerate(lvl_indices):
                jitter = torch.rand((indices.shape[0], self.DIM), dtype=torch.float32, device=indices.device)
                x = self._cell_points(lvl, indices, jitter)
                occ = occ_eval_fn(x).squeeze(-1)
                self._ema_update(lvl, indices, occ, ema_decay)
        self._rebinarize(occ_thre)

    def _cell_points(self, lvl: int, indices: Tensor, jitter: Tensor) -> Tensor:
        if not indices.is_cuda:
            unit = (self.grid_coords[indices] + jitter) / self.resolution
            return self.aabbs[lvl, :3] + unit * (self.aabbs[lvl, 3:] - self.aabbs[lvl, :3])
        n = indices.shape[0]
        x = torch.empty((n, self.DIM), dtype=torch.float32, device=indices.device)
        res = (C.c_int32 * 3)(*[int(v) for v in self.binaries.shape[1:]])
        with torch.cuda.device(indices.device):
            B.call("nfa_grid_cell_points", B.ptr(indices.contiguous()), B.ptr(jitter.contiguous()), n, res,
                   self.aabbs.data_ptr() + 24 * lvl, B.ptr(x), B.stream())
        return x

    def _ema_update(self, lvl: int, indices: Tensor, occ: Tensor, ema_decay: float) -> None:
        if not self.occs.is_cuda:
            cell_ids = lvl * self.cells_per_lvl + indices
            self.occs[cell_ids] = torch.maximum(self.occs[cell_ids] * ema_decay, occ)
            return
        n = indices.shape[0]
        occ = occ.to(torch.float32).contiguous()
        assert occ.shape == (n,), "occ_eval_fn must return one value per position"
        scratch = torch.empty(n, dtype=torch.float32, device=self.occs.device)
        with torch.cuda.device(self.occs.device):
            B.call("nfa_grid_ema_update", B.ptr(self.occs), lvl * self.cells_per_lvl, B.ptr(indices.contiguous()), n, B.ptr(occ),
                   float(ema_decay), B.ptr(scratch), B.stream())
        self._occs_mean_cache = None

    def _rebinarize(self, occ_thre: float) -> None:
        if not self.occs.is_cuda:
            thre = torch.clamp(self.occs[self.occs >= 0].mean(), max=occ_thre)
            self.binaries = (self.occs > thre).view(self.binaries.shape)
            return
        from ..grid import _walk_supported
        dev = self.occs.device
        shape = tuple(self.binaries.shape)
        if not _walk_supported(self.binaries):
            thre = torch.clamp(self.occs[self.occs >= 0].mean(), max=occ_thre)
            self.binaries = (self.occs > thre).view(self.binaries.shape)
            return
        res = (C.c_int32 * 3)(*shape[1:])
        binaries = torch.empty(shape, dtype=torch.bool, device=dev)
        bits = torch.empty(int(B.load().nfa_walk_bits_words(shape[0], res)), dtype=torch.int32, device=dev)
        scratch = torch.empty(int(B.load().nfa_grid_rebinarize_scratch_bytes()) // 8 + 1, dtype=torch.float64, device=dev)
        with torch.cuda.device(dev):
            B.call("nfa_grid_rebinarize", B.ptr(self.occs), shape[0], res, float(occ_thre), B.ptr(binaries), B.ptr(bits),
                   B.ptr(scratch), B.stream())
        binaries._nfa_walk_bits = (binaries._version, bits)
        self.binaries = binaries
        self._occs_mean_cache = None


_PINNED_READ = __import__("os").environ.get("NERFACC_AMD_PINNED_READ", "1") != "0"
_PINNED_TOTALS: dict = {}


def _pinned_total(dev) -> Tensor:
    buf = _PINNED_TOTALS.get(dev.index)
    if buf is None:
        buf = _PINNED_TOTALS[dev.index] = torch.empty(1, dtype=torch.int64, pin_memory=True)
    return buf


_KEPT_FRACTION: dict = {}
_SPECULATE_COMPACTION = __import__("os").environ.get("NERFACC_AMD_SPECULATE_COMPACTION", "1") != "0"


def _compact(seg: SegInfo, vis: Tensor, cnts: Tensor, t_starts: Tensor, t_ends: Tensor):
    dev = t_starts.device
    n = t_starts.numel()
    key = (seg.n_rays, dev.index)
    with torch.cuda.device(dev):
        total = torch.empty(1, dtype=torch.int64, device=dev)
        out_starts = _exclusive_cumsum(cnts, total)
        frac = _KEPT_FRACTION.get(key, 1.0) if _SPECULATE_COMPACTION else 1.0
        host = _pinned_total(dev)
        ri = ts = te = None
        cap = 0

        def run(ri, ts, te, capacity):
            B.call("nfa_compact_samples", B.ptr(vis), B.ptr(t_starts), B.ptr(t_ends), B.ptr(seg.packed_info),
                   B.ptr(seg.tiles), seg.n_tiles, B.ptr(out_starts), seg.n_rays, n, B.ptr(ri), B.ptr(ts), B.ptr(te), capacity, B.stream())

        if frac < 1.0 and n > 0:
            cap = min(n, ((int(n * min(1.0, frac * 1.03)) + 8192) // 4096) * 4096)
            main = torch.cuda.current_stream()
            ready = torch.cuda.Event(); ready.record(main)
            from ..grid import _side_stream
            side = _side_stream(dev)
            with torch.cuda.stream(side):
                side.wait_event(ready)
                host.copy_(total, non_blocking=True)
                done = torch.cuda.Event(); done.record(side)
            ri = torch.empty(cap, dtype=torch.int64, device=dev)
            ts = torch.empty(cap, dtype=torch.float32, device=dev)
            te = torch.empty(cap, dtype=torch.float32, device=dev)
            run(ri, ts, te, cap)
            done.synchronize()
            m = int(host[0])
        elif _PINNED_READ:
            host.copy_(total, non_blocking=True)
            done = torch.cuda.Event(); done.record()
            done.synchronize()
            m = int(host[0])
        else:
            m = int(total.item())
        if n > 0:
            _KEPT_FRACTION[key] = m / n
        if m == n:
            return None
        if cap > 0 and m <= cap:
            ri, ts, te = ri[:m], ts[:m], te[:m]
        else:
            ri = torch.empty(m, dtype=torch.int64, device=dev)
            ts = torch.empty(m, dtype=torch.float32, device=dev)
            te = torch.empty(m, dtype=torch.float32, device=dev)
            if m > 0:
                run(ri, ts, te, m)
        step = const_step_of(t_starts, t_ends)
        if step is not None:
            tag_const_step(ts, te, step)
        packed = torch.stack([out_starts, cnts], dim=-1)
    info = tag_trusted(packed, m)
    tag_ray_indices(ri, seg.n_rays, info)
    return ri, ts, te


def _meshgrid3d(res: Tensor, device: Union[torch.device, str] = "cpu") -> Tensor:
    assert len(res) == 3
    axes = [torch.arange(int(r), dtype=torch.long) for r in res.tolist()]
    return torch.stack(torch.meshgrid(axes, indexing="ij"), dim=-1).to(device)
```

nerfacc_amd/grid.py:

```python
from __future__ import annotations

import ctypes as C
import os
from typing import Optional, Tuple

import torch
from torch import Tensor

from . import _backend as B
from ._segments import tag_const_step, tag_ray_indices, tag_trusted
from .data_specs import RayIntervals, RaySamples


@torch.no_grad()
def ray_aabb_intersect(
    rays_o: Tensor,
    rays_d: Tensor,
    aabbs: Tensor,
    near_plane: float = -float("inf"),
    far_plane: float = float("inf"),
    miss_value: float = float("inf"),
) -> Tuple[Tensor, Tensor, Tensor]:
    assert rays_o.ndim == 2 and rays_o.shape[-1] == 3
    assert rays_d.ndim == 2 and rays_d.shape[-1] == 3
    assert aabbs.ndim == 2 and aabbs.shape[-1] == 6
    dev = B.require_device(rays_o, rays_d, aabbs)
    rays_o, rays_d, aabbs = rays_o.float().contiguous(), rays_d.float().contiguous(), aabbs.float().contiguous()
    n, m = rays_o.shape[0], aabbs.shape[0]
    t_mins = torch.empty((n, m), dtype=torch.float32, device=dev)
    t_maxs = torch.empty((n, m), dtype=torch.float32, device=dev)
    hits = torch.empty((n, m), dtype=torch.bool, device=dev)
    with torch.cuda.device(dev):
        B.call("nfa_ray_aabb_intersect", B.ptr(rays_o), B.ptr(rays_d), n, B.ptr(aabbs), m, float(near_plane),
               float(far_plane), float(miss_value), B.ptr(t_mins), B.ptr(t_maxs), B.ptr(hits), B.stream())
    return t_mins, t_maxs, hits


def _traverse_args(rays_o, rays_d, rays_mask, binaries, aabbs, t_sorted, t_indices, hits, near_planes, far_planes,
                   step_size, cone_angle, limit, mode) -> B.TraverseArgs:
    a = B.TraverseArgs()
    a.n_rays = rays_o.shape[0]
    a.rays_o, a.rays_d, a.rays_mask = B.ptr(rays_o), B.ptr(rays_d), B.ptr(rays_mask)
    a.n_grids = binaries.shape[0]
    a.res[0], a.res[1], a.res[2] = binaries.shape[1], binaries.shape[2], binaries.shape[3]
    a.binaries, a.aabbs = B.ptr(binaries), B.ptr(aabbs)
    a.hits, a.t_sorted, a.t_indices = B.ptr(hits), B.ptr(t_sorted), B.ptr(t_indices)
    a.near_planes, a.far_planes = B.ptr(near_planes), B.ptr(far_planes)
    a.step_size, a.cone_angle = float(step_size), float(cone_angle)
    a.traverse_steps_limit, a.mode = int(limit), int(mode)
    bricks, coarse = _get_bricks(binaries)
    a._keepalive = (bricks, coarse)
    a.bricks, a.coarse = B.ptr(bricks), B.ptr(coarse)
    return a


def _launch(a: B.TraverseArgs) -> None:
    B.call("nfa_traverse_grids", C.byref(a), B.stream())


def _exclusive_cumsum(cnts: Tensor, total_out: Tensor):
    starts = torch.empty_like(cnts)
    scratch = B.cumsum_scratch(cnts.numel(), cnts.device)
    B.call("nfa_exclusive_cumsum_i64", B.ptr(cnts), cnts.numel(), B.ptr(starts), B.ptr(total_out), B.ptr(scratch),
           B.stream())
    return starts


def _cumsum_packed(cnts: Tensor, total_out: Tensor, stats: bool = False) -> Tensor:
    packed = torch.empty((cnts.numel(), 2), dtype=torch.int64, device=cnts.device)
    scratch = B.cumsum_scratch(cnts.numel(), cnts.device)
    B.call("nfa_exclusive_cumsum_pairs_stats_i64" if stats else "nfa_exclusive_cumsum_pairs_i64", B.ptr(cnts), cnts.numel(),
           B.ptr(packed), B.ptr(total_out), B.ptr(scratch), B.stream())
    return packed


MAX_EVENT_LEVELS = 8


def ray_events(rays_o: Tensor, rays_d: Tensor, aabbs: Tensor):
    G = aabbs.shape[0]
    if G > MAX_EVENT_LEVELS or not rays_o.is_cuda:
        t_mins, t_maxs, hits = ray_aabb_intersect(rays_o, rays_d, aabbs)
        t_sorted, t_indices = torch.sort(torch.cat([t_mins, t_maxs], dim=-1), dim=-1)
        return t_sorted, t_indices, hits
    dev = B.require_device(rays_o, rays_d, aabbs)
    rays_o, rays_d, aabbs = rays_o.float().contiguous(), rays_d.float().contiguous(), aabbs.float().contiguous()
    n = rays_o.shape[0]
    t_sorted = torch.empty((n, 2 * G), dtype=torch.float32, device=dev)
    t_indices = torch.empty((n, 2 * G), dtype=torch.int64, device=dev)
    hits = torch.empty((n, G), dtype=torch.bool, device=dev)
    with torch.cuda.device(dev):
        B.call("nfa_ray_events", B.ptr(rays_o), B.ptr(rays_d), n, B.ptr(aabbs), G, B.ptr(t_sorted), B.ptr(t_indices),
               B.ptr(hits), B.stream())
    return t_sorted, t_indices, hits


def _prepare(rays_o, rays_d, binaries, aabbs, near_planes, far_planes, rays_mask, t_sorted, t_indices, hits,
             allow_fused: bool):
    dev = B.require_device(rays_o, rays_d, binaries, aabbs)
    assert rays_o.ndim == 2 and rays_o.shape[-1] == 3 and rays_d.shape == rays_o.shape
    assert binaries.ndim == 4 and aabbs.ndim == 2 and aabbs.shape == (binaries.shape[0], 6)
    rays_o, rays_d, aabbs = rays_o.float().contiguous(), rays_d.float().contiguous(), aabbs.float().contiguous()
    binaries = (binaries if binaries.dtype == torch.bool else binaries.bool()).contiguous()
    n_rays = rays_o.shape[0]
    if near_planes is None:
        near_planes = torch.zeros(n_rays, dtype=torch.float32, device=dev)
    if far_planes is None:
        far_planes = torch.full((n_rays,), float("inf"), dtype=torch.float32, device=dev)
    near_planes, far_planes = near_planes.float().contiguous(), far_planes.float().contiguous()
    if rays_mask is not None:
        rays_mask = rays_mask.bool().contiguous()
    if t_sorted is None or t_indices is None or hits is None:
        if allow_fused and binaries.shape[0] == 1:
            t_sorted = t_indices = hits = None
        else:
            t_sorted, t_indices, hits = ray_events(rays_o, rays_d, aabbs)
    if t_sorted is not None:
        t_sorted = t_sorted.float().contiguous()
        t_indices = t_indices.to(torch.int64).contiguous()
        hits = hits.bool().contiguous()
    return dev, rays_o, rays_d, binaries, aabbs, near_planes, far_planes, rays_mask, t_sorted, t_indices, hits


@torch.no_grad()
def traverse_grids(
    rays_o: Tensor,
    rays_d: Tensor,
    binaries: Tensor,
    aabbs: Tensor,
    near_planes: Optional[Tensor] = None,
    far_planes: Optional[Tensor] = None,
    step_size: Optional[float] = 1e-3,
    cone_angle: Optional[float] = 0.0,
    traverse_steps_limit: Optional[int] = None,
    over_allocate: Optional[bool] = False,
    rays_mask: Optional[Tensor] = None,
    t_sorted: Optional[Tensor] = None,
    t_indices: Optional[Tensor] = None,
    hits: Optional[Tensor] = None,
) -> Tuple[RayIntervals, RaySamples, Tensor]:
    near_hint = 0.0 if near_planes is None else None
    if traverse_steps_limit is None:
        traverse_steps_limit = -1
    if over_allocate:
        assert traverse_steps_limit > 0, "traverse_steps_limit must be set if over_allocate is True."
    (dev, rays_o, rays_d, binaries, aabbs, near_planes, far_planes, rays_mask, t_sorted, t_indices,
     hits) = _prepare(rays_o, rays_d, binaries, aabbs, near_planes, far_planes, rays_mask, t_sorted, t_indices, hits,
                      allow_fused=True)
    n_rays = rays_o.shape[0]
    i64 = dict(dtype=torch.int64, device=dev)
    with torch.cuda.device(dev):
        terminate = torch.empty(n_rays, dtype=torch.float32, device=dev)
        totals = torch.empty(2, **i64)
        iv_packed = sm_packed = None
        if over_allocate:
            limit = int(traverse_steps_limit)
            mask_l = torch.ones(n_rays, **i64) if rays_mask is None else rays_mask.to(torch.int64)
            sm_alloc = mask_l * limit
            iv_alloc = sm_alloc * 2
            sm_off = torch.cumsum(sm_alloc, 0) - sm_alloc
            iv_off = sm_off * 2
            n_alive = int(mask_l.sum().item()) if rays_mask is not None else n_rays
            n_sm, n_iv = n_alive * limit, n_alive * limit * 2
            iv_cnts, sm_cnts = torch.empty(n_rays, **i64), torch.empty(n_rays, **i64)
            iv_vals = torch.zeros(n_iv, dtype=torch.float32, device=dev)
            iv_ri = torch.zeros(n_iv, **i64)
            iv_l = torch.zeros(n_iv, dtype=torch.bool, device=dev)
            iv_r = torch.zeros(n_iv, dtype=torch.bool, device=dev)
            sm_vals = torch.zeros(n_sm, dtype=torch.float32, device=dev)
            sm_ri = torch.zeros(n_sm, **i64)
            sm_valid = torch.zeros(n_sm, dtype=torch.bool, device=dev)
            a = _traverse_args(rays_o, rays_d, rays_mask, binaries, aabbs, t_sorted, t_indices, hits, near_planes,
                               far_planes, step_size, cone_angle, limit, 2)
            a.iv_vals, a.iv_ray_indices, a.iv_is_left, a.iv_is_right = B.ptr(iv_vals), B.ptr(iv_ri), B.ptr(iv_l), B.ptr(iv_r)
            a.iv_starts, a.iv_cnts = B.ptr(iv_off), B.ptr(iv_cnts)
            a.sm_vals, a.sm_ray_indices, a.sm_is_valid = B.ptr(sm_vals), B.ptr(sm_ri), B.ptr(sm_valid)
            a.sm_starts, a.sm_cnts = B.ptr(sm_off), B.ptr(sm_cnts)
            a.terminate_planes = B.ptr(terminate)
            _launch(a)
            iv_starts = _exclusive_cumsum(iv_cnts, totals[0:1])
            sm_starts = _exclusive_cumsum(sm_cnts, totals[1:2])
        elif float(step_size) > 0.0 and float(cone_angle) == 0.0 and _walk_supported(binaries):
            iv_cnts, sm_cnts = torch.empty(n_rays, **i64), torch.empty(n_rays, **i64)
            meta = torch.zeros(3, **i64)
            a = _traverse_args(rays_o, rays_d, None, binaries, aabbs, t_sorted, t_indices, hits, near_planes,
                               far_planes, step_size, cone_angle, traverse_steps_limit, 0)
            a.iv_cnts, a.sm_cnts, a.terminate_planes = B.ptr(iv_cnts), B.ptr(sm_cnts), B.ptr(terminate)
            bits = _get_walk_bits(binaries)
            run_cnts = torch.empty(n_rays, dtype=torch.int32, device=dev)
            runs = torch.empty((MAX_RUNS, n_rays), dtype=torch.int64, device=dev)
            while True:
                B.call("nfa_traverse_runs", C.byref(a), B.ptr(bits), B.ptr(run_cnts), B.ptr(runs), MAX_RUNS,
                       B.ptr(meta[2:3]), float("nan") if near_hint is None else near_hint, None, 0, B.stream())
                iv_packed = _cumsum_packed(iv_cnts, meta[0:1])
                sm_packed = _cumsum_packed(sm_cnts, meta[1:2])
                n_iv, n_sm, n_overflow = (int(v) for v in meta.tolist())
                n_overflow, off_lattice = n_overflow & 0xFFFFFFFF, n_overflow >> 32
                if not off_lattice or near_hint is None:
                    break
                near_hint = None
                meta.zero_()
            iv_vals = torch.empty(n_iv, dtype=torch.float32, device=dev)
            iv_ri = torch.empty(n_iv, **i64)
            iv_l = torch.empty(n_iv, dtype=torch.bool, device=dev)
            iv_r = torch.empty(n_iv, dtype=torch.bool, device=dev)
            sm_vals = torch.empty(n_sm, dtype=torch.float32, device=dev)
            sm_ri = torch.empty(n_sm, **i64)
            sm_valid = torch.ones(n_sm, dtype=torch.bool, device=dev)
            if n_sm > 0:
                B.call("nfa_expand_runs", n_rays, float(step_size), B.ptr(run_cnts), B.ptr(runs), MAX_RUNS, B.ptr(sm_packed),
                       None, None, B.ptr(sm_vals), B.ptr(sm_ri), n_sm, B.stream())
                B.call("nfa_expand_intervals", n_rays, float(step_size), B.ptr(run_cnts), B.ptr(runs), MAX_RUNS,
                       B.ptr(iv_packed), B.ptr(iv_vals), B.ptr(iv_ri), B.ptr(iv_l), B.ptr(iv_r), B.stream())
                if n_overflow > 0:
                    iv_starts, sm_starts = iv_packed[:, 0].contiguous(), sm_packed[:, 0].contiguous()
                    a.mode = 1
                    a.terminate_planes = None
                    a.iv_vals, a.iv_ray_indices, a.iv_is_left, a.iv_is_right = (B.ptr(iv_vals), B.ptr(iv_ri), B.ptr(iv_l),
                                                                                 B.ptr(iv_r))
                    a.iv_starts = B.ptr(iv_starts)
                    a.sm_vals, a.sm_ray_indices, a.sm_is_valid = B.ptr(sm_vals), B.ptr(sm_ri), B.ptr(sm_valid)
                    a.sm_starts = B.ptr(sm_starts)
                    a.ray_filter, a.ray_filter_min = B.ptr(run_cnts), MAX_RUNS
                    _launch(a)
        else:
            iv_cnts, sm_cnts = torch.empty(n_rays, **i64), torch.empty(n_rays, **i64)
            a = _traverse_args(rays_o, rays_d, None, binaries, aabbs, t_sorted, t_indices, hits, near_planes,
                               far_planes, step_size, cone_angle, traverse_steps_limit, 0)
            a.iv_cnts, a.sm_cnts, a.terminate_planes = B.ptr(iv_cnts), B.ptr(sm_cnts), B.ptr(terminate)
            _launch(a)
            iv_starts = _exclusive_cumsum(iv_cnts, totals[0:1])
            sm_starts = _exclusive_cumsum(sm_cnts, totals[1:2])
            n_iv, n_sm = (int(v) for v in totals.tolist())
            iv_vals = torch.empty(n_iv, dtype=torch.float32, device=dev)
            iv_ri = torch.empty(n_iv, **i64)
            iv_l = torch.empty(n_iv, dtype=torch.bool, device=dev)
            iv_r = torch.empty(n_iv, dtype=torch.bool, device=dev)
            sm_vals = torch.empty(n_sm, dtype=torch.float32, device=dev)
            sm_ri = torch.empty(n_sm, **i64)
            sm_valid = torch.empty(n_sm, dtype=torch.bool, device=dev)
            if n_sm > 0:
                a.mode = 1
                a.terminate_planes = None
                a.iv_vals, a.iv_ray_indices, a.iv_is_left, a.iv_is_right = B.ptr(iv_vals), B.ptr(iv_ri), B.ptr(iv_l), B.ptr(iv_r)
                a.iv_starts = B.ptr(iv_starts)
                a.sm_vals, a.sm_ray_indices, a.sm_is_valid = B.ptr(sm_vals), B.ptr(sm_ri), B.ptr(sm_valid)
                a.sm_starts = B.ptr(sm_starts)
                _launch(a)
        if iv_packed is None:
            iv_packed = torch.stack([iv_starts, iv_cnts], dim=-1)
            sm_packed = torch.stack([sm_starts, sm_cnts], dim=-1)
    if not over_allocate:
        tag_trusted(iv_packed, n_iv)
        info = tag_trusted(sm_packed, n_sm)
        tag_ray_indices(sm_ri, n_rays, info)
    intervals = RayIntervals(vals=iv_vals, packed_info=iv_packed, ray_indices=iv_ri, is_left=iv_l, is_right=iv_r)
    samples = RaySamples(vals=sm_vals, packed_info=sm_packed, ray_indices=sm_ri, is_valid=sm_valid)
    return intervals, samples, terminate


MAX_RUNS = int(os.environ.get("NERFACC_AMD_MAX_RUNS", "32"))


def _get_bricks(binaries: Tensor):
    cached = getattr(binaries, "_nfa_bricks", None)
    if cached is not None and cached[0] == binaries._version:
        return cached[1], cached[2]
    dev = binaries.device
    res = (C.c_int32 * 3)(*binaries.shape[1:])
    words = int(B.load().nfa_bricks_words(binaries.shape[0], res))
    bricks = torch.empty(words, dtype=torch.int64, device=dev)
    coarse = torch.empty((words + 31) // 32, dtype=torch.int32, device=dev)
    B.call("nfa_pack_bricks", B.ptr(binaries), binaries.shape[0], res, B.ptr(bricks), B.ptr(coarse), B.stream())
    try:
        binaries._nfa_bricks = (binaries._version, bricks, coarse)
    except Exception:
        pass
    return bricks, coarse


WALK_MAX_RES = 512


def _walk_supported(binaries: Tensor) -> bool:
    if max(binaries.shape[1:]) > WALK_MAX_RES:
        return False
    res = (C.c_int32 * 3)(*binaries.shape[1:])
    return int(B.load().nfa_walk_bits_words(binaries.shape[0], res)) * 32 < (1 << 31)


def _get_walk_bits(binaries: Tensor) -> Tensor:
    cached = getattr(binaries, "_nfa_walk_bits", None)
    if cached is not None and cached[0] == binaries._version:
        return cached[1]
    res = (C.c_int32 * 3)(*binaries.shape[1:])
    words = int(B.load().nfa_walk_bits_words(binaries.shape[0], res))
    bits = torch.empty(words, dtype=torch.int32, device=binaries.device)
    B.call("nfa_pack_walk_bits", B.ptr(binaries), binaries.shape[0], res, B.ptr(bits), B.stream())
    try:
        binaries._nfa_walk_bits = (binaries._version, bits)
    except Exception:
        pass
    return bits


_SIDE_STREAMS: dict = {}


def _side_stream(dev) -> "torch.cuda.Stream":
    key = (dev.index, torch.cuda.current_stream(dev).cuda_stream)
    st = _SIDE_STREAMS.get(key)
    if st is None:
        st = _SIDE_STREAMS[key] = torch.cuda.Stream(device=dev)
    return st


SPECULATE = os.environ.get("NERFACC_AMD_SPECULATE", "1") != "0"
_SPEC_CAPACITY: dict = {}
_PINNED: dict = {}


def _pinned_meta(dev) -> Tensor:
    buf = _PINNED.get(dev.index)
    if buf is None:
        buf = _PINNED[dev.index] = torch.empty(8, dtype=torch.int64, pin_memory=True)
    return buf


CONE_RUNS = os.environ.get("NERFACC_AMD_CONE_RUNS", "1") != "0"
ALIVE_LIST_FRACTION = float(os.environ.get("NERFACC_AMD_ALIVE_FRACTION", "0.75"))
CONE_WALK = os.environ.get("NERFACC_AMD_CONE_WALK", "1") != "0"
CONE_ARENA = os.environ.get("NERFACC_AMD_CONE_ARENA", "1") != "0"
CONE_ARENA_MIN = 4096
CONE_BIN_THRESHOLD = 1.25


@torch.no_grad()
def _traverse_samples(rays_o, rays_d, binaries, aabbs, near_planes, far_planes, step_size, cone_angle,
                      rays_mask=None, traverse_steps_limit=None, t_sorted=None, t_indices=None, hits=None,
                      return_terminate=False, near_hint=None, bin_rays=False, stats_sink=None, speculate=True, n_alive=None,
                      alive_list=None):
    limit = -1 if traverse_steps_limit is None else int(traverse_steps_limit)
    use_runs = float(step_size) > 0.0 and float(cone_angle) == 0.0 and _walk_supported(binaries)
    use_cone_runs = CONE_RUNS and float(step_size) > 0.0 and float(cone_angle) > 0.0
    if (rays_mask is not None or limit > 0) and (not (use_runs or use_cone_runs) or (use_cone_runs and limit <= 0)):
        iv, sm, term = traverse_grids(rays_o, rays_d, binaries, aabbs, near_planes, far_planes, step_size, cone_angle,
                                      limit if limit > 0 else None, limit > 0, rays_mask, t_sorted, t_indices, hits)
        valid = sm.is_valid if sm.is_valid is not None else torch.ones_like(sm.ray_indices, dtype=torch.bool)
        out = (sm.ray_indices[valid], iv.vals[iv.is_left], iv.vals[iv.is_right], sm.packed_info)
        return (*out, term) if return_terminate else out
    (dev, rays_o, rays_d, binaries, aabbs, near_planes, far_planes, rays_mask, t_sorted, t_indices,
     hits) = _prepare(rays_o, rays_d, binaries, aabbs, near_planes, far_planes, rays_mask, t_sorted, t_indices, hits,
                      allow_fused=True)
    n_rays = rays_o.shape[0]
    with torch.cuda.device(dev):
        masked = rays_mask is not None or limit > 0
        spec_key = (n_rays, dev.index)
        binned = bool(bin_rays) and n_rays >= 4096
        alive = None
        if (alive_list is not None and n_alive is not None and rays_mask is not None and (use_runs or use_cone_runs) and not binned
                and 0 <= n_alive <= alive_list.numel() and alive_list.dtype == torch.int32 and alive_list.device == dev):
            alive = alive_list[:int(n_alive)]
            sm_cnts = torch.zeros(n_rays, dtype=torch.int64, device=dev)
            terminate = near_planes.clone() if return_terminate else None
        elif (rays_mask is not None and n_alive is not None and (use_runs or use_cone_runs) and not binned
                and 0 <= n_alive and n_alive < ALIVE_LIST_FRACTION * n_rays):
            alive = torch.nonzero_static(rays_mask, size=int(n_alive)).view(-1).to(torch.int32)
            sm_cnts = torch.zeros(n_rays, dtype=torch.int64, device=dev)
            terminate = near_planes.clone() if return_terminate else None
        else:
            sm_cnts = torch.empty(n_rays, dtype=torch.int64, device=dev)
            terminate = torch.empty(n_rays, dtype=torch.float32, device=dev) if return_terminate else None
        meta = torch.zeros(6, dtype=torch.int64, device=dev)
        a = _traverse_args(rays_o, rays_d, rays_mask, binaries, aabbs, t_sorted, t_indices, hits, near_planes, far_planes,
                           step_size, cone_angle, limit, 2 if ((use_runs or use_cone_runs) and masked) else 0)
        a.sm_cnts = B.ptr(sm_cnts)
        a.terminate_planes = B.ptr(terminate)
        if use_runs:
            bits = _get_walk_bits(binaries)
            run_cnts = (torch.zeros if alive is not None else torch.empty)(n_rays, dtype=torch.int32, device=dev)
            runs = torch.empty((MAX_RUNS, n_rays), dtype=torch.int64, device=dev)
            order = alive
            if binned:
                order = torch.empty(n_rays, dtype=torch.int32, device=dev)
                scratch = torch.empty(1024 + n_rays, dtype=torch.uint8, device=dev)
                B.call("nfa_bin_rays", B.ptr(rays_o), B.ptr(rays_d), n_rays, B.ptr(aabbs[-1]), B.ptr(order), B.ptr(scratch),
                       B.stream())
            B.call("nfa_traverse_runs", C.byref(a), B.ptr(bits), B.ptr(run_cnts), B.ptr(runs), MAX_RUNS,
                   B.ptr(meta[3:4]), float("nan") if near_hint is None else float(near_hint), B.ptr(order),
                   0 if order is None else order.numel(), B.stream())
        elif use_cone_runs:
            _get_bricks(binaries)
            arena, arena_cap = None, 0
            run_cnts = (torch.zeros if alive is not None else torch.empty)(n_rays, dtype=torch.int32, device=dev)
            runs = torch.empty((MAX_RUNS, n_rays), dtype=torch.int64, device=dev)
            order = alive
            if binned or (bin_rays is None and n_rays >= 65536 and alive is None and limit <= 0):
                order = torch.empty(n_rays, dtype=torch.int32, device=dev)
                scratch = torch.empty(1024 + n_rays, dtype=torch.uint8, device=dev)
                res3 = (C.c_int32 * 3)(*binaries.shape[1:])
                B.call("nfa_bin_rays_levels", B.ptr(rays_o), B.ptr(rays_d), n_rays, B.ptr(aabbs), binaries.shape[0], res3,
                       float(near_hint) if near_hint is not None else 0.0, B.ptr(order), B.ptr(scratch), B.ptr(meta[4:6]), B.stream())
                if not binned and not (stats_sink is not None and stats_sink.get("cells_max_over_mean", 1.0) > CONE_BIN_THRESHOLD):
                    order = None
            if CONE_WALK and _walk_supported(binaries) and min(binaries.shape[1:]) >= 4:
                arena_cap = CONE_ARENA and max(CONE_ARENA_MIN, (n_rays // 8 + 15) // 16 * 16)
                arena = torch.zeros(2 * arena_cap, dtype=torch.int64, device=dev) if arena_cap else None
                B.call("nfa_traverse_cone_walk", C.byref(a), B.ptr(_get_walk_bits(binaries)), B.ptr(run_cnts), B.ptr(runs), MAX_RUNS,
                       B.ptr(meta[3:4]), B.ptr(arena), arena_cap, B.ptr(order), 0 if order is None else order.numel(), B.stream())
            else:
                B.call("nfa_traverse_cone_runs", C.byref(a), B.ptr(run_cnts), B.ptr(runs), MAX_RUNS, B.ptr(meta[3:4]), B.ptr(order),
                       0 if order is None else order.numel(), B.stream())
        else:
            _launch(a)
        packed_info = _cumsum_packed(sm_cnts, meta[0:3], stats=True)
        cap = _SPEC_CAPACITY.get(spec_key, 0) if (SPECULATE and speculate and use_runs) else 0
        t_starts = t_ends = ray_indices = None
        if cap > 0:
            host = _pinned_meta(dev)
            main = torch.cuda.current_stream()
            ready = torch.cuda.Event(); ready.record(main)
            side = _side_stream(dev)
            with torch.cuda.stream(side):
                side.wait_event(ready)
                host[:6].copy_(meta, non_blocking=True)
                done = torch.cuda.Event(); done.record(side)
            t_starts = torch.empty(cap, dtype=torch.float32, device=dev)
            t_ends = torch.empty(cap, dtype=torch.float32, device=dev)
            ray_indices = torch.empty(cap, dtype=torch.int64, device=dev)
            B.call("nfa_expand_runs", n_rays, float(step_size), B.ptr(run_cnts), B.ptr(runs), MAX_RUNS,
                   B.ptr(packed_info), B.ptr(t_starts), B.ptr(t_ends), None, B.ptr(ray_indices), cap, B.stream())
            done.synchronize()
            n_sm, s_max, s_sum, n_overflow, c_max, c_sum = (int(v) for v in host[:6].tolist())
        else:
            n_sm, s_max, s_sum, n_overflow, c_max, c_sum = (int(v) for v in meta.tolist())
        n_overflow, off_lattice = n_overflow & 0xFFFFFFFF, n_overflow >> 32
        n_arena = 0
        if use_cone_runs and arena is not None:
            n_arena, off_lattice = min(off_lattice, arena_cap), 0
        if off_lattice and use_runs and near_hint is not None:
            return _traverse_samples(rays_o, rays_d, binaries, aabbs, near_planes, far_planes, step_size, cone_angle,
                                     rays_mask=rays_mask, traverse_steps_limit=traverse_steps_limit, t_sorted=t_sorted,
                                     t_indices=t_indices, hits=hits, return_terminate=return_terminate, near_hint=None,
                                     bin_rays=bin_rays, stats_sink=stats_sink, speculate=speculate, n_alive=n_alive,
                                     alive_list=alive_list)
        if stats_sink is not None and c_sum > 0:
            stats_sink["cells_max_over_mean"] = 64.0 * c_max / c_sum
        if SPECULATE and use_runs:
            _SPEC_CAPACITY[spec_key] = ((int(n_sm * 1.03) + 4096) // 4096) * 4096
        if stats_sink is not None and s_sum > 0:
            stats_sink["max_over_mean"] = 64.0 * s_max / s_sum
        expanded = cap > 0 and n_sm <= cap
        if expanded:
            t_starts, t_ends, ray_indices = t_starts[:n_sm], t_ends[:n_sm], ray_indices[:n_sm]
        else:
            t_starts = torch.empty(n_sm, dtype=torch.float32, device=dev)
            t_ends = torch.empty(n_sm, dtype=torch.float32, device=dev)
            ray_indices = torch.empty(n_sm, dtype=torch.int64, device=dev)
        if n_sm > 0:
            main = torch.cuda.current_stream()
            joined = None
            if (use_runs or use_cone_runs) and n_overflow > 0:
                sm_starts = packed_info[:, 0].contiguous()
                side = _side_stream(dev)
                side.wait_stream(main)
                with torch.cuda.stream(side):
                    a.mode = 1
                    a.terminate_planes = None
                    a.sm_starts = B.ptr(sm_starts)
                    a.sm_t_starts, a.sm_t_ends, a.sm_ray_indices = B.ptr(t_starts), B.ptr(t_ends), B.ptr(ray_indices)
                    a.ray_filter, a.ray_filter_min = B.ptr(run_cnts), MAX_RUNS
                    _launch(a)
                    joined = torch.cuda.Event()
                    joined.record(side)
            if use_runs and not expanded:
                B.call("nfa_expand_runs", n_rays, float(step_size), B.ptr(run_cnts), B.ptr(runs), MAX_RUNS,
                       B.ptr(packed_info), B.ptr(t_starts), B.ptr(t_ends), None, B.ptr(ray_indices), n_sm, B.stream())
            elif use_cone_runs:
                B.call("nfa_expand_cone_runs", n_rays, float(step_size), float(cone_angle), B.ptr(run_cnts), B.ptr(runs),
                       MAX_RUNS, B.ptr(packed_info), B.ptr(t_starts), B.ptr(t_ends), B.ptr(ray_indices), B.stream())
                if n_arena > 0:
                    B.call("nfa_expand_cone_arena", B.ptr(arena), n_arena, float(step_size), float(cone_angle), B.ptr(packed_info),
                           B.ptr(t_starts), B.ptr(t_ends), B.ptr(ray_indices), B.stream())
            if joined is not None:
                main.wait_event(joined)
            if not (use_runs or use_cone_runs):
                a.mode = 1
                a.terminate_planes = None
                sm_starts = packed_info[:, 0].contiguous()
                a.sm_starts = B.ptr(sm_starts)
                a.sm_t_starts, a.sm_t_ends = B.ptr(t_starts), B.ptr(t_ends)
                a.sm_ray_indices = None
                _launch(a)
                B.call("nfa_fill_ray_indices", n_rays, B.ptr(packed_info), B.ptr(ray_indices), B.stream())
    info = tag_trusted(packed_info, n_sm)
    tag_ray_indices(ray_indices, n_rays, info)
    if use_runs and not masked:
        tag_const_step(t_starts, t_ends, step_size)
    out = (ray_indices, t_starts, t_ends, packed_info)
    return (*out, terminate) if return_terminate else out


def _enlarge_aabb(aabb: Tensor, factor: float) -> Tensor:
    center = (aabb[:3] + aabb[3:]) / 2
    extent = (aabb[3:] - aabb[:3]) / 2
    return torch.cat([center - extent * factor, center + extent * factor])


def _query(x: Tensor, data: Tensor, base_aabb: Tensor) -> Tuple[Tensor, Tensor]:
    lo, hi = base_aabb[:3], base_aabb[3:]
    u = (x - lo) / (hi - lo)
    r = (u - 0.5).abs().amax(dim=-1).clamp_min(0.1)
    mip = (torch.frexp(r)[1].long() + 1).clamp_min(0)
    inside = mip < data.shape[0]
    uu = (u - 0.5) / (2 ** mip)[:, None] + 0.5
    res = torch.tensor(data.shape[1:], device=x.device)
    ix = torch.minimum((uu * res).long(), res - 1)
    lvl = mip.clamp_max(data.shape[0] - 1)
    return data[lvl, ix[:, 0], ix[:, 1], ix[:, 2]] * inside, inside
```

Before: 755.6 million rays/s.

## Fuse per-ray cumsum and segment tile-table build into single-pass bookkeeping kernel

Replaces the two-launch exclusive cumsum plus separate segment-tile construction with a single decoupled-lookback kernel. It computes per-ray offsets, stats and the tile lookup table in one pass, falling back to the old path if the bounded spin-wait times out. The compaction check is also changed: when no compaction is expected, a cheap sum of kept counts replaces the full cumsum before deciding to skip compaction. This aims to remove kernel launches and a separate tile-build pass, at the cost of inter-block spin waits that rely on blocks being co-resident.

Result: faster. 763.4 million rays/s, median of 6 (+1.0%).

```diff
diff --git a/include/nerfacc_hip.h b/include/nerfacc_hip.h
--- a/include/nerfacc_hip.h
+++ b/include/nerfacc_hip.h
@@ -33,6 +33,11 @@
                                    void *scratch, nfa_stream_t stream);
 int nfa_exclusive_cumsum_pairs_stats_i64(const int64_t *cnts, int64_t n, int64_t *packed_info ,
                                          int64_t *total_and_stats , void *scratch, nfa_stream_t stream);
+int nfa_sum_i64(const int64_t *x, int64_t n, int64_t *sum, nfa_stream_t stream);
+int64_t nfa_ray_bookkeeping_state_words(int64_t n);
+int nfa_ray_bookkeeping(const int64_t *cnts, int64_t n, int64_t tile_elems, int64_t tiles_rows_cap, int64_t *state,
+                        int64_t *packed_info , int64_t *total_and_stats , int64_t *tiles ,
+                        nfa_stream_t stream);
 
 int nfa_pack_info(const int64_t *ray_indices, int64_t n, int64_t n_rays, int64_t *packed_info ,
                   int32_t *flags , void *scratch, nfa_stream_t stream);
diff --git a/nerfacc_amd/_backend.py b/nerfacc_amd/_backend.py
--- a/nerfacc_amd/_backend.py
+++ b/nerfacc_amd/_backend.py
@@ -37,6 +37,9 @@
     "nfa_exclusive_cumsum_i64": [_vp, _i64, _vp, _vp, _vp, _vp],
     "nfa_exclusive_cumsum_pairs_i64": [_vp, _i64, _vp, _vp, _vp, _vp],
     "nfa_exclusive_cumsum_pairs_stats_i64": [_vp, _i64, _vp, _vp, _vp, _vp],
+    "nfa_sum_i64": [_vp, _i64, _vp, _vp],
+    "nfa_ray_bookkeeping_state_words": [_i64],
+    "nfa_ray_bookkeeping": [_vp, _i64, _i64, _i64, _vp, _vp, _vp, _vp, _vp],
     "nfa_pack_info": [_vp, _i64, _i64, _vp, _vp, _vp, _vp],
     "nfa_pdf_loss_fwd": [_vp, _vp, _vp, _vp, _i64, _i32, _i32, _f32, _vp, _vp, _vp],
     "nfa_pdf_loss_bwd": [_vp, _vp, _vp, _i64, _i32, _i32, _f32, _vp, _vp, _vp, _vp],
@@ -161,7 +164,7 @@
     "nfa_set_tuning": [C.c_char_p, C.c_char_p],
     "nfa_device_arch": [C.c_char_p, _int],
 }
-_RESTYPES = {"nfa_grid_rebinarize_scratch_bytes": _i64, "nfa_hashgrid_sorted_scratch_bytes": _i64, "nfa_hashgrid_sorted_scratch_bytes_d": _i64, "nfa_planereg_partials": _i64, "nfa_vmreg_partials": _i64, "nfa_bricks_words": _i64, "nfa_walk_bits_words": _i64, "nfa_pdf_loss_partials": _i64, "nfa_cumsum_scratch_bytes": _i64, "nfa_seg_table_rows": _i64, "nfa_seg_plan": None, "nfa_last_error": C.c_char_p}
+_RESTYPES = {"nfa_grid_rebinarize_scratch_bytes": _i64, "nfa_hashgrid_sorted_scratch_bytes": _i64, "nfa_hashgrid_sorted_scratch_bytes_d": _i64, "nfa_planereg_partials": _i64, "nfa_vmreg_partials": _i64, "nfa_bricks_words": _i64, "nfa_walk_bits_words": _i64, "nfa_pdf_loss_partials": _i64, "nfa_cumsum_scratch_bytes": _i64, "nfa_ray_bookkeeping_state_words": _i64, "nfa_seg_table_rows": _i64, "nfa_seg_plan": None, "nfa_last_error": C.c_char_p}
 
 EXPORTED_SYMBOLS = tuple(_SIGS)
 
diff --git a/nerfacc_amd/_segments.py b/nerfacc_amd/_segments.py
--- a/nerfacc_amd/_segments.py
+++ b/nerfacc_amd/_segments.py
@@ -21,6 +21,7 @@
     sorted_indices: bool = True
     n_tiles: int = 0
     trusted: bool = False
+    zero_word: Optional[Tensor] = None
 
 
 _ATTR = "_nfa_seg"
@@ -58,6 +59,14 @@
 
 def tag_trusted(packed_info: Tensor, n_elems: int) -> SegInfo:
     return seginfo_from_packed(packed_info, n_elems, trusted=True)
+
+
+def tag_trusted_tiles(packed_info: Tensor, n_elems: int, tiles: Tensor, n_tiles: int) -> SegInfo:
+    rows = int(B.load().nfa_seg_table_rows(n_tiles))
+    assert tiles.shape[0] >= rows and packed_info.dtype == torch.int64 and packed_info.is_contiguous()
+    info = SegInfo(packed_info, packed_info.shape[0], n_elems, tiles[:rows], True, n_tiles=n_tiles, trusted=True)
+    setattr(packed_info, _ATTR, (packed_info._version, n_elems, info))
+    return info
 
 
 def pack_info_native(ray_indices: Tensor, n_rays: int):
diff --git a/nerfacc_amd/csrc/grid.hip b/nerfacc_amd/csrc/grid.hip
--- a/nerfacc_amd/csrc/grid.hip
+++ b/nerfacc_amd/csrc/grid.hip
@@ -1,6 +1,7 @@
 #include <stdarg.h>
 
 #include "common.hip.h"
+#include "seg_tiles.h"
 #include "march.h"
 
 namespace nfa {
@@ -494,6 +495,155 @@
     return NFA_OK;
 }
 
+constexpr int SUM_PAIRS = 16;
+constexpr int SUM_BLOCK = CS_THREADS * SUM_PAIRS * 2;
+__global__ __launch_bounds__(CS_THREADS) void sum_i64_kernel(const int64_t *__restrict__ x, int64_t n, unsigned long long *__restrict__ sum)
+{
+    __shared__ int64_t lds[8];
+    const int64_t base = (int64_t)blockIdx.x * SUM_BLOCK;
+    int64_t s = 0;
+    if ((reinterpret_cast<uintptr_t>(x) & 15) == 0 && base + SUM_BLOCK <= n) {
+        const longlong2 *x2 = reinterpret_cast<const longlong2 *>(x + base);
+        longlong2 v[SUM_PAIRS];
+#pragma unroll
+        for (int k = 0; k < SUM_PAIRS; ++k) v[k] = x2[k * CS_THREADS + threadIdx.x];
+#pragma unroll
+        for (int k = 0; k < SUM_PAIRS; ++k) s += v[k].x + v[k].y;
+    } else {
+#pragma unroll 8
+        for (int k = 0; k < 2 * SUM_PAIRS; ++k) {
+            const int64_t i = base + (int64_t)k * CS_THREADS + threadIdx.x;
+            s += i < n ? x[i] : 0;
+        }
+    }
+    int64_t tot;
+    block_excl_scan_i64(s, tot, lds);
+    if (threadIdx.x == 0 && tot != 0) atomicAdd(sum, (unsigned long long)tot);
+}
+
+constexpr int BK_FAULT = 0, BK_TICKET = 1, BK_SUMS = 2;
+constexpr unsigned long long BK_READY = 1ull << 63;
+constexpr int BK_WAVES = 16, BK_THREADS = 64 * BK_WAVES;
+constexpr int BK_GROUPS = BK_THREADS / CS_THREADS;
+constexpr int BK_CHUNK = BK_THREADS * CS_ITEMS;
+constexpr int64_t BK_MAX_CHUNKS = 2048 / BK_GROUPS;
+constexpr int BK_MAX_POLLS = 4096;
+
+__device__ __forceinline__ int64_t bk_block_excl_scan(int64_t v, int64_t &block_total, int64_t *lds )
+{
+    const int lane = lane_id(), wave = threadIdx.x >> 6;
+    const int64_t incl = wave_incl_sum_i64(v);
+    if (lane == 63) lds[wave] = incl;
+    __syncthreads();
+    int64_t wave_off = 0, tot = 0;
+#pragma unroll
+    for (int w = 0; w < BK_WAVES; ++w) {
+        const int64_t x = lds[w];
+        if (w < wave) wave_off += x;
+        tot += x;
+    }
+    __syncthreads();
+    block_total = tot;
+    return wave_off + incl - v;
+}
+
+__global__ __launch_bounds__(BK_THREADS) void ray_bookkeeping_kernel(const int64_t *__restrict__ cnts, int64_t n, SegTileSize tile_elems,
+                                                                      int64_t rows_cap, unsigned long long *state,
+                                                                      longlong2 *__restrict__ packed, int64_t *__restrict__ total_and_stats,
+                                                                      longlong2 *__restrict__ tiles)
+{
+    __shared__ int64_t lds[BK_WAVES];
+    __shared__ int64_t ticket;
+    __shared__ int fault;
+    if (threadIdx.x == 0) {
+        ticket = (int64_t)__hip_atomic_fetch_add(&state[BK_TICKET], 1ull, __ATOMIC_RELAXED, __HIP_MEMORY_SCOPE_AGENT);
+        fault = 0;
+    }
+    __syncthreads();
+    const int64_t c = ticket;
+    if (c >= (int64_t)gridDim.x) {
+        if (threadIdx.x == 0) __hip_atomic_store(&state[BK_FAULT], 1ull, __ATOMIC_RELAXED, __HIP_MEMORY_SCOPE_AGENT);
+        return;
+    }
+    const int64_t base = c * BK_CHUNK + (int64_t)threadIdx.x * CS_ITEMS;
+    int64_t v[CS_ITEMS];
+    int64_t s = 0;
+#pragma unroll
+    for (int k = 0; k < CS_ITEMS; ++k) {
+        v[k] = (base + k < n) ? cnts[base + k] : 0;
+        s += v[k];
+    }
+    const int64_t v_prev = (base > 0 && base < n) ? cnts[base - 1] : 0;
+    int64_t tot;
+    int64_t run = bk_block_excl_scan(s, tot, lds);
+    if (threadIdx.x == 0)
+        __hip_atomic_store(&state[BK_SUMS + c], BK_READY | (unsigned long long)tot, __ATOMIC_RELAXED, __HIP_MEMORY_SCOPE_AGENT);
+    int64_t before = 0;
+    if ((int64_t)threadIdx.x < c) {
+        unsigned long long w = 0;
+        int polls = 0;
+        for (;;) {
+            w = __hip_atomic_load(&state[BK_SUMS + threadIdx.x], __ATOMIC_RELAXED, __HIP_MEMORY_SCOPE_AGENT);
+            if ((w & BK_READY) || ++polls >= BK_MAX_POLLS) break;
+            __builtin_amdgcn_s_sleep(8);
+        }
+        if (w & BK_READY) before = (int64_t)(w & ~BK_READY);
+        else fault = 1;
+    }
+    int64_t block_off;
+    bk_block_excl_scan(before, block_off, lds);
+    if (fault) {
+#pragma unroll
+        for (int k = 0; k < CS_ITEMS; ++k)
+            if (base + k < n) packed[base + k] = make_longlong2(0, 0);
+        if (threadIdx.x == 0) __hip_atomic_store(&state[BK_FAULT], 1ull, __ATOMIC_RELAXED, __HIP_MEMORY_SCOPE_AGENT);
+        return;
+    }
+    run += block_off;
+    if ((c & 1) == 0 && threadIdx.x < CS_THREADS) {
+        int64_t m = 0;
+#pragma unroll
+        for (int k = 0; k < CS_ITEMS; ++k) m = v[k] > m ? v[k] : m;
+        for (int off = 1; off < 8; off <<= 1) { const int64_t u = __shfl_xor(m, off, 64); m = u > m ? u : m; }
+        int64_t gm = (lane_id() & 7) == 0 ? m : 0;
+        int64_t ws = s;
+        for (int off = 8; off < 64; off <<= 1) gm += __shfl_xor(gm, off, 64);
+        for (int off = 1; off < 64; off <<= 1) ws += __shfl_xor(ws, off, 64);
+        unsigned long long *stats = reinterpret_cast<unsigned long long *>(total_and_stats + 1);
+        if (lane_id() == 0) { atomicAdd(&stats[0], (unsigned long long)gm); atomicAdd(&stats[1], (unsigned long long)ws); }
+    }
+    const int64_t last_row = rows_cap - 1;
+    int64_t s_prev = base > 0 ? run - v_prev : -1;
+#pragma unroll
+    for (int k = 0; k < CS_ITEMS; ++k) {
+        const int64_t r = base + k;
+        if (r < n) {
+            packed[r] = make_longlong2(run, v[k]);
+            seg_tile_write(tiles, seg_tile_span_ray(r, run, s_prev, tile_elems), r, last_row);
+            if (r == n - 1) {
+                const int64_t total = run + v[k];
+                total_and_stats[0] = total;
+                const int64_t n_tiles = tile_elems.tile_of(total) + n / SEG_TILE_ROWS + 1;
+                seg_tile_write(tiles, seg_tile_span_sentinel(n, run, v[k], n_tiles, tile_elems), n, last_row);
+            }
+        }
+        s_prev = run;
+        run += v[k];
+    }
+}
+
+__global__ __launch_bounds__(256) void seg_build_tiles_dev_kernel(const longlong2 *__restrict__ packed, int64_t n, SegTileSize tile_elems,
+                                                                  int64_t rows_cap, const int64_t *__restrict__ total,
+                                                                  longlong2 *__restrict__ tiles)
+{
+    const int64_t last_row = rows_cap - 1;
+    for (int64_t r = (int64_t)blockIdx.x * blockDim.x + threadIdx.x; r <= n; r += (int64_t)blockDim.x * gridDim.x) {
+        const longlong2 prev = r > 0 ? packed[r - 1] : make_longlong2(-1, 0);
+        if (r < n) seg_tile_write(tiles, seg_tile_span_ray(r, packed[r].x, prev.x, tile_elems), r, last_row);
+        else seg_tile_write(tiles, seg_tile_span_sentinel(n, prev.x, prev.y, seg_n_tiles(*total, n, tile_elems.elems), tile_elems), n, last_row);
+    }
+}
+
 __global__ __launch_bounds__(256) void pack_hist_kernel(const int64_t *__restrict__ ray_indices, int64_t n,
                                                         int64_t n_rays, unsigned long long *__restrict__ packed,
                                                         int32_t *__restrict__ flags)
@@ -594,6 +744,49 @@
                 "exclusive_cumsum_pairs_stats_i64: bad arguments");
     return run_cumsum(cnts, n, 1, packed_info, 1, total_and_stats, scratch, as_stream(stream),
                       reinterpret_cast<unsigned long long *>(total_and_stats + 1));
+}
+
+int nfa_sum_i64(const int64_t *x, int64_t n, int64_t *sum, nfa_stream_t stream)
+{
+    NFA_REQUIRE(n >= 0 && sum && (n == 0 || x), "sum_i64: bad arguments");
+    if (n == 0) return NFA_OK;
+    hipLaunchKernelGGL(sum_i64_kernel, dim3((unsigned)ceil_div64(n, SUM_BLOCK)), dim3(CS_THREADS), 0, as_stream(stream), x, n,
+                       reinterpret_cast<unsigned long long *>(sum));
+    NFA_CHECK_LAUNCH("sum_i64");
+    return NFA_OK;
+}
+
+int64_t nfa_ray_bookkeeping_state_words(int64_t n)
+{
+    const int64_t groups = ceil_div64(n > 0 ? n : 1, CS_BLOCK);
+    return BK_SUMS + groups + 1;
+}
+
+int nfa_ray_bookkeeping(const int64_t *cnts, int64_t n, int64_t tile_elems, int64_t tiles_rows_cap, int64_t *state,
+                        int64_t *packed_info, int64_t *total_and_stats, int64_t *tiles, nfa_stream_t stream)
+{
+    NFA_REQUIRE(n >= 0 && n < ((int64_t)1 << 31) - 64 && state && total_and_stats && tiles && tiles_rows_cap >= 0 &&
+                    (n == 0 || (cnts && packed_info)),
+                "ray_bookkeeping: bad arguments");
+    NFA_REQUIRE(tile_elems >= 64 && tile_elems % 4 == 0, "ray_bookkeeping: tile_elems must be a multiple of 4 (>= 64)");
+    if (n == 0) return NFA_OK;
+    hipStream_t s = as_stream(stream);
+    const int64_t chunks = ceil_div64(n, BK_CHUNK);
+    if (chunks <= BK_MAX_CHUNKS) {
+        hipLaunchKernelGGL(ray_bookkeeping_kernel, dim3((unsigned)chunks), dim3(BK_THREADS), 0, s, cnts, n, seg_tile_size(tile_elems), tiles_rows_cap,
+                           reinterpret_cast<unsigned long long *>(state), reinterpret_cast<longlong2 *>(packed_info), total_and_stats,
+                           reinterpret_cast<longlong2 *>(tiles));
+        NFA_CHECK_LAUNCH("ray_bookkeeping");
+        return NFA_OK;
+    }
+    const int rc = run_cumsum(cnts, n, 1, packed_info, 1, total_and_stats, state + BK_SUMS, s,
+                              reinterpret_cast<unsigned long long *>(total_and_stats + 1));
+    if (rc != NFA_OK) return rc;
+    hipLaunchKernelGGL(seg_build_tiles_dev_kernel, dim3(grid_1d(n + 1, 256)), dim3(256), 0, s,
+                       reinterpret_cast<const longlong2 *>(packed_info), n, seg_tile_size(tile_elems), tiles_rows_cap, total_and_stats,
+                       reinterpret_cast<longlong2 *>(tiles));
+    NFA_CHECK_LAUNCH("ray_bookkeeping");
+    return NFA_OK;
 }
 
 int nfa_pack_info(const int64_t *ray_indices, int64_t n, int64_t n_rays, int64_t *packed_info, int32_t *flags,
diff --git a/nerfacc_amd/csrc/seg_tiles.h b/nerfacc_amd/csrc/seg_tiles.h
--- /dev/null
+++ b/nerfacc_amd/csrc/seg_tiles.h
@@ -0,0 +1,51 @@
+#pragma once
+#include <hip/hip_runtime.h>
+#include <stdint.h>
+
+namespace nfa {
+
+#ifndef NFA_SEG_TILE_ROWS
+#define NFA_SEG_TILE_ROWS 256
+#endif
+constexpr int64_t SEG_TILE_ROWS = NFA_SEG_TILE_ROWS;
+
+__host__ __device__ inline int64_t seg_n_tiles(int64_t n_elems, int64_t n_rays, int64_t tile_elems)
+{
+    return n_elems / tile_elems + (n_rays > 0 ? n_rays : 0) / SEG_TILE_ROWS + 1;
+}
+__host__ __device__ inline int64_t seg_table_rows(int64_t n_tiles) { return n_tiles + 1; }
+
+struct SegTileSize {
+    int64_t elems;
+    int shift;
+    __host__ __device__ inline int64_t tile_of(int64_t e ) const { return shift >= 0 ? e >> shift : e / elems; }
+};
+inline SegTileSize seg_tile_size(int64_t tile_elems)
+{
+    int shift = -1;
+    if (tile_elems > 0 && (tile_elems & (tile_elems - 1)) == 0)
+        for (shift = 0; ((int64_t)1 << shift) < tile_elems;) ++shift;
+    return SegTileSize{tile_elems, shift};
+}
+
+struct SegTileSpan { int64_t b_lo, b_hi, e_first; };
+
+__host__ __device__ inline int64_t seg_tile_first_row(int64_t r, int64_t s_prev, const SegTileSize &t)
+{
+    return (s_prev < 0) ? 0 : t.tile_of(s_prev) + (r - 1) / SEG_TILE_ROWS + 1;
+}
+__host__ __device__ inline SegTileSpan seg_tile_span_ray(int64_t r, int64_t s, int64_t s_prev, const SegTileSize &t)
+{
+    return SegTileSpan{seg_tile_first_row(r, s_prev, t), t.tile_of(s) + r / SEG_TILE_ROWS, s};
+}
+__host__ __device__ inline SegTileSpan seg_tile_span_sentinel(int64_t n_rays, int64_t s_prev, int64_t n_prev, int64_t n_tiles,
+                                                              const SegTileSize &t)
+{
+    return SegTileSpan{seg_tile_first_row(n_rays, s_prev, t), n_tiles, (s_prev < 0) ? 0 : s_prev + n_prev};
+}
+__device__ __forceinline__ void seg_tile_write(longlong2 *__restrict__ tiles, const SegTileSpan &sp, int64_t r, int64_t last_row)
+{
+    for (int64_t b = sp.b_lo; b <= sp.b_hi && b <= last_row; ++b) tiles[b] = make_longlong2(r, sp.e_first);
+}
+
+}
diff --git a/nerfacc_amd/csrc/segscan.hip b/nerfacc_amd/csrc/segscan.hip
--- a/nerfacc_amd/csrc/segscan.hip
+++ b/nerfacc_amd/csrc/segscan.hip
@@ -2,16 +2,13 @@
 
 #include "common.hip.h"
 #include "samples.h"
+#include "seg_tiles.h"
 
 namespace nfa {
 
 constexpr int SE = 4;
 constexpr int SQ = SE / 4;
 constexpr int SEG_CHUNK = 64 * SE;
-#ifndef NFA_SEG_TILE_ROWS
-#define NFA_SEG_TILE_ROWS 256
-#endif
-constexpr int64_t SEG_TILE_ROWS = NFA_SEG_TILE_ROWS;
 #ifndef NFA_VIS_EXP_FREE
 #define NFA_VIS_EXP_FREE 1
 #endif
@@ -21,12 +18,12 @@
 constexpr int SEG_WAVES_PER_BLOCK = NFA_SEG_WAVES_PER_BLOCK;
 
 __global__ __launch_bounds__(256) void seg_build_tiles_kernel(const int64_t *__restrict__ packed_info, int64_t n_rays,
-                                                              int64_t n_elems, int64_t tile_elems, int64_t n_tiles,
+                                                              int64_t n_elems, SegTileSize tile_elems, int64_t n_tiles,
                                                               longlong2 *__restrict__ tiles, int32_t *__restrict__ flags)
 {
     for (int64_t r = (int64_t)blockIdx.x * blockDim.x + threadIdx.x; r <= n_rays;
          r += (int64_t)blockDim.x * gridDim.x) {
-        int64_t b_lo, b_hi, e_first;
+        SegTileSpan sp;
         bool bad = false;
         if (r < n_rays) {
             const int64_t s = packed_info[2 * r], n = packed_info[2 * r + 1];
@@ -38,22 +35,17 @@
             }
             bad |= (n < 0) || (s < 0) || (s + n > n_elems);
             if (bad) { if (flags) atomicOr(flags, 1); continue; }
-            b_lo = (s_prev < 0) ? 0 : s_prev / tile_elems + (r - 1) / SEG_TILE_ROWS + 1;
-            b_hi = s / tile_elems + r / SEG_TILE_ROWS;
-            e_first = s;
+            sp = seg_tile_span_ray(r, s, s_prev, tile_elems);
         } else {
             const int64_t s_prev = n_rays > 0 ? packed_info[2 * n_rays - 2] : -1;
             const int64_t n_prev = n_rays > 0 ? packed_info[2 * n_rays - 1] : 0;
-            b_lo = (s_prev < 0) ? 0 : s_prev / tile_elems + (n_rays - 1) / SEG_TILE_ROWS + 1;
-            b_hi = n_tiles;
-            e_first = (s_prev < 0) ? 0 : s_prev + n_prev;
+            sp = seg_tile_span_sentinel(n_rays, s_prev, n_prev, n_tiles, tile_elems);
             if (s_prev > n_elems) { if (flags) atomicOr(flags, 1); continue; }
         }
-        for (int64_t b = b_lo; b <= b_hi && b <= n_tiles; ++b) tiles[b] = make_longlong2(r, e_first);
-    }
-}
-
-__host__ __device__ inline int64_t seg_table_rows(int64_t n_tiles) { return n_tiles + 1; }
+        seg_tile_write(tiles, sp, r, n_tiles);
+    }
+}
+
 
 struct F4 { float v[SE]; };
 
@@ -2169,7 +2161,7 @@
     const int64_t t_env = tuning_env("NFA_SEG_TILE") ? atoll(tuning_env("NFA_SEG_TILE")) : 0;
     const int64_t t = t_env > 0 ? t_env : 1024;
     *tile_elems = t;
-    *n_tiles = n_elems / t + (n_rays > 0 ? n_rays : 0) / SEG_TILE_ROWS + 1;
+    *n_tiles = seg_n_tiles(n_elems, n_rays, t);
 }
 
 int64_t nfa_seg_table_rows(int64_t n_tiles) { return seg_table_rows(n_tiles); }
@@ -2180,12 +2172,12 @@
     NFA_REQUIRE(n_rays >= 0 && n_elems >= 0 && tiles, "seg_build_tiles: bad arguments");
     NFA_REQUIRE(n_rays == 0 || packed_info, "seg_build_tiles: packed_info is null");
     NFA_REQUIRE(n_rays < ((int64_t)1 << 31) - 64, "seg_build_tiles: too many rays");
-    NFA_REQUIRE(tile_elems >= 64 && tile_elems % 4 == 0 && n_tiles == n_elems / tile_elems + n_rays / SEG_TILE_ROWS + 1,
+    NFA_REQUIRE(tile_elems >= 64 && tile_elems % 4 == 0 && n_tiles == seg_n_tiles(n_elems, n_rays, tile_elems),
                 "seg_build_tiles: tile_elems must be a multiple of 4 (>= 64) and n_tiles what nfa_seg_plan returns for (n_elems, n_rays)");
     hipStream_t s = as_stream(stream);
     if (flags && hipMemsetAsync(flags, 0, sizeof(int32_t), s) != hipSuccess) { set_error("seg_build_tiles: memset failed"); return NFA_EHIP; }
     hipLaunchKernelGGL(seg_build_tiles_kernel, dim3(grid_1d(n_rays + 1, 256)), dim3(256), 0, s, packed_info, n_rays,
-                       n_elems, tile_elems, n_tiles, reinterpret_cast<longlong2 *>(tiles), flags);
+                       n_elems, seg_tile_size(tile_elems), n_tiles, reinterpret_cast<longlong2 *>(tiles), flags);
     NFA_CHECK_LAUNCH("seg_build_tiles");
     return NFA_OK;
 }
diff --git a/nerfacc_amd/estimators/occ_grid.py b/nerfacc_amd/estimators/occ_grid.py
--- a/nerfacc_amd/estimators/occ_grid.py
+++ b/nerfacc_amd/estimators/occ_grid.py
@@ -165,6 +165,9 @@
         if (alpha_thre > 0.0 or early_stop_eps > 0.0) and (sigma_fn is not None or alpha_fn is not None):
             alpha_thre = min(alpha_thre, self._occs_mean())
             seg: SegInfo = tag_trusted(packed_info, t_starts.numel())
+            kept_word, seg.zero_word = seg.zero_word, None
+            if kept_word is None:
+                kept_word = torch.zeros(1, dtype=torch.int64, device=t_starts.device)
             if sigma_fn is not None:
                 if t_starts.shape[0] != 0:
                     sigmas = sigma_fn(t_starts, t_ends, ray_indices)
@@ -180,7 +183,7 @@
                     alphas = torch.empty((0,), device=t_starts.device)
                 assert alphas.shape == t_starts.shape, "alphas must have shape of (N,)! Got {}".format(alphas.shape)
                 vis, cnts = _visibility_native(seg, None, None, alphas, None, early_stop_eps, alpha_thre, True)
-            compacted = _compact(seg, vis, cnts, t_starts, t_ends)
+            compacted = _compact(seg, vis, cnts, t_starts, t_ends, kept_word)
             if compacted is not None:
                 ray_indices, t_starts, t_ends = compacted
         return ray_indices, t_starts, t_ends
@@ -366,14 +369,30 @@
 _SPECULATE_COMPACTION = __import__("os").environ.get("NERFACC_AMD_SPECULATE_COMPACTION", "1") != "0"
 
 
-def _compact(seg: SegInfo, vis: Tensor, cnts: Tensor, t_starts: Tensor, t_ends: Tensor):
+def _read_word(word: Tensor) -> int:
+    if not _PINNED_READ:
+        return int(word.item())
+    host = _pinned_total(word.device)
+    host.copy_(word, non_blocking=True)
+    done = torch.cuda.Event(); done.record()
+    done.synchronize()
+    return int(host[0])
+
+
+def _compact(seg: SegInfo, vis: Tensor, cnts: Tensor, t_starts: Tensor, t_ends: Tensor, kept_word: Optional[Tensor] = None):
     dev = t_starts.device
     n = t_starts.numel()
     key = (seg.n_rays, dev.index)
     with torch.cuda.device(dev):
+        frac = _KEPT_FRACTION.get(key, 1.0) if _SPECULATE_COMPACTION else 1.0
+        if kept_word is not None and not (frac < 1.0 and n > 0):
+            B.call("nfa_sum_i64", B.ptr(cnts), cnts.numel(), B.ptr(kept_word), B.stream())
+            if _read_word(kept_word) == n:
+                if n > 0:
+                    _KEPT_FRACTION[key] = 1.0
+                return None
         total = torch.empty(1, dtype=torch.int64, device=dev)
         out_starts = _exclusive_cumsum(cnts, total)
-        frac = _KEPT_FRACTION.get(key, 1.0) if _SPECULATE_COMPACTION else 1.0
         host = _pinned_total(dev)
         ri = ts = te = None
         cap = 0
@@ -398,13 +417,8 @@
             run(ri, ts, te, cap)
             done.synchronize()
             m = int(host[0])
-        elif _PINNED_READ:
-            host.copy_(total, non_blocking=True)
-            done = torch.cuda.Event(); done.record()
-            done.synchronize()
-            m = int(host[0])
         else:
-            m = int(total.item())
+            m = _read_word(total)
         if n > 0:
             _KEPT_FRACTION[key] = m / n
         if m == n:
diff --git a/nerfacc_amd/grid.py b/nerfacc_amd/grid.py
--- a/nerfacc_amd/grid.py
+++ b/nerfacc_amd/grid.py
@@ -2,13 +2,14 @@
 
 import ctypes as C
 import os
+import warnings
 from typing import Optional, Tuple
 
 import torch
 from torch import Tensor
 
 from . import _backend as B
-from ._segments import tag_const_step, tag_ray_indices, tag_trusted
+from ._segments import tag_const_step, tag_ray_indices, tag_trusted, tag_trusted_tiles
 from .data_specs import RayIntervals, RaySamples
 
 
@@ -72,6 +73,37 @@
     B.call("nfa_exclusive_cumsum_pairs_stats_i64" if stats else "nfa_exclusive_cumsum_pairs_i64", B.ptr(cnts), cnts.numel(),
            B.ptr(packed), B.ptr(total_out), B.ptr(scratch), B.stream())
     return packed
+
+
+META_HOST_WORDS = 8
+META_SPARE = 6
+META_STATE = 7
+
+
+def _ray_bookkeeping(sm_cnts: Tensor, meta: Tensor, table_cap: int):
+    n_rays = sm_cnts.numel()
+    tile_elems, n_tiles_cap = B.seg_plan(table_cap, n_rays)
+    rows_cap = int(B.load().nfa_seg_table_rows(n_tiles_cap))
+    packed = torch.empty((n_rays, 2), dtype=torch.int64, device=sm_cnts.device)
+    tiles = torch.empty((rows_cap, 2), dtype=torch.int64, device=sm_cnts.device)
+    B.call("nfa_ray_bookkeeping", B.ptr(sm_cnts), n_rays, tile_elems, rows_cap, B.ptr(meta[META_STATE:]), B.ptr(packed),
+           B.ptr(meta[0:3]), B.ptr(tiles), B.stream())
+    return packed, tiles
+
+
+def _settle_bookkeeping(words, sm_cnts: Tensor, packed_info: Tensor, tiles: Tensor, table_cap: int):
+    words = list(words)
+    if words[META_STATE] != 0:
+        warnings.warn("nerfacc_amd: nfa_ray_bookkeeping gave up a bounded wait; the per-ray offsets are recomputed by the "
+                      "two-launch scan", RuntimeWarning, stacklevel=3)
+        again = torch.zeros(3, dtype=torch.int64, device=sm_cnts.device)
+        packed_info = _cumsum_packed(sm_cnts, again, stats=True)
+        words[0:3] = [int(v) for v in again.tolist()]
+        words[META_STATE] = 0
+        return packed_info, None, words, True
+    if words[0] > table_cap:
+        tiles = None
+    return packed_info, tiles, words, False
 
 
 MAX_EVENT_LEVELS = 8
@@ -371,7 +403,7 @@
         else:
             sm_cnts = torch.empty(n_rays, dtype=torch.int64, device=dev)
             terminate = torch.empty(n_rays, dtype=torch.float32, device=dev) if return_terminate else None
-        meta = torch.zeros(6, dtype=torch.int64, device=dev)
+        meta = torch.zeros(META_STATE + int(B.load().nfa_ray_bookkeeping_state_words(n_rays)), dtype=torch.int64, device=dev)
         a = _traverse_args(rays_o, rays_d, rays_mask, binaries, aabbs, t_sorted, t_indices, hits, near_planes, far_planes,
                            step_size, cone_angle, limit, 2 if ((use_runs or use_cone_runs) and masked) else 0)
         a.sm_cnts = B.ptr(sm_cnts)
@@ -413,7 +445,13 @@
                        0 if order is None else order.numel(), B.stream())
         else:
             _launch(a)
-        packed_info = _cumsum_packed(sm_cnts, meta[0:3], stats=True)
+        table_cap = (_SPEC_CAPACITY.get(spec_key, 0)
+                     if (SPECULATE and (use_runs or use_cone_runs) and not masked and n_rays > 0) else 0)
+        tiles = None
+        if table_cap > 0:
+            packed_info, tiles = _ray_bookkeeping(sm_cnts, meta, table_cap)
+        else:
+            packed_info = _cumsum_packed(sm_cnts, meta[0:3], stats=True)
         cap = _SPEC_CAPACITY.get(spec_key, 0) if (SPECULATE and speculate and use_runs) else 0
         t_starts = t_ends = ray_indices = None
         if cap > 0:
@@ -423,7 +461,7 @@
             side = _side_stream(dev)
             with torch.cuda.stream(side):
                 side.wait_event(ready)
-                host[:6].copy_(meta, non_blocking=True)
+                host[:META_HOST_WORDS].copy_(meta[:META_HOST_WORDS], non_blocking=True)
                 done = torch.cuda.Event(); done.record(side)
             t_starts = torch.empty(cap, dtype=torch.float32, device=dev)
             t_ends = torch.empty(cap, dtype=torch.float32, device=dev)
@@ -431,9 +469,13 @@
             B.call("nfa_expand_runs", n_rays, float(step_size), B.ptr(run_cnts), B.ptr(runs), MAX_RUNS,
                    B.ptr(packed_info), B.ptr(t_starts), B.ptr(t_ends), None, B.ptr(ray_indices), cap, B.stream())
             done.synchronize()
-            n_sm, s_max, s_sum, n_overflow, c_max, c_sum = (int(v) for v in host[:6].tolist())
-        else:
-            n_sm, s_max, s_sum, n_overflow, c_max, c_sum = (int(v) for v in meta.tolist())
+            words = [int(v) for v in host[:META_HOST_WORDS].tolist()]
+        else:
+            words = [int(v) for v in meta[:META_HOST_WORDS].tolist()]
+        redone = False
+        if tiles is not None:
+            packed_info, tiles, words, redone = _settle_bookkeeping(words, sm_cnts, packed_info, tiles, table_cap)
+        n_sm, s_max, s_sum, n_overflow, c_max, c_sum = words[:6]
         n_overflow, off_lattice = n_overflow & 0xFFFFFFFF, n_overflow >> 32
         n_arena = 0
         if use_cone_runs and arena is not None:
@@ -446,11 +488,11 @@
                                      alive_list=alive_list)
         if stats_sink is not None and c_sum > 0:
             stats_sink["cells_max_over_mean"] = 64.0 * c_max / c_sum
-        if SPECULATE and use_runs:
+        if SPECULATE and (use_runs or (use_cone_runs and not masked)):
             _SPEC_CAPACITY[spec_key] = ((int(n_sm * 1.03) + 4096) // 4096) * 4096
         if stats_sink is not None and s_sum > 0:
             stats_sink["max_over_mean"] = 64.0 * s_max / s_sum
-        expanded = cap > 0 and n_sm <= cap
+        expanded = cap > 0 and n_sm <= cap and not redone
         if expanded:
             t_starts, t_ends, ray_indices = t_starts[:n_sm], t_ends[:n_sm], ray_indices[:n_sm]
         else:
@@ -493,7 +535,11 @@
                 a.sm_ray_indices = None
                 _launch(a)
                 B.call("nfa_fill_ray_indices", n_rays, B.ptr(packed_info), B.ptr(ray_indices), B.stream())
-    info = tag_trusted(packed_info, n_sm)
+    if tiles is not None:
+        info = tag_trusted_tiles(packed_info, n_sm, tiles, B.seg_plan(n_sm, n_rays)[1])
+    else:
+        info = tag_trusted(packed_info, n_sm)
+    info.zero_word = meta[META_SPARE:META_SPARE + 1]
     tag_ray_indices(ray_indices, n_rays, info)
     if use_runs and not masked:
         tag_const_step(t_starts, t_ends, step_size)
```
